# Dorothy-2016/rgbd360

Measured on AMD Instinct MI355X. Metric: registered Frame360 pairs/sec @ 8×640×480; ICP-reduce HBM GB/s vs roofline, higher is better.
Workload: dtype f32

## Files before the change

### include/rgbd360_hip.h

```cpp
#ifndef RGBD360_HIP_H
#define RGBD360_HIP_H
#include <stddef.h>
#include <stdint.h>

#ifdef __cplusplus
extern "C" {
#endif

#define R360_NUM_SENSORS 8
#define R360_MAX_PYR 6

typedef struct r360_ctx r360_ctx;
typedef struct r360_calib r360_calib;
typedef struct r360_frame r360_frame;

int         r360_ctx_create(int device, r360_ctx** out);
void        r360_ctx_destroy(r360_ctx* ctx);
int         r360_ctx_sync(r360_ctx* ctx);
void*       r360_ctx_stream(r360_ctx* ctx);
const char* r360_last_error(void);
const char* r360_version(void);
const char* r360_data_dir(void);

int  r360_calib_create(r360_ctx* ctx, int rows, int cols, r360_calib** out);
void r360_calib_destroy(r360_calib* c);
int  r360_calib_set_extrinsics(r360_calib* c, const float* rt8);
int  r360_calib_get_extrinsics(const r360_calib* c, float* rt8, float* rt_inv8, float K[9]);
int  r360_calib_load_extrinsics(r360_calib* c, const char* dir);
int  r360_calib_load_intrinsics(r360_calib* c, const char* dir);
int  r360_calib_create_sphere(r360_ctx* ctx, int sph_rows, int sph_cols, r360_calib** out);

enum {
    R360_BUILD_UNDISTORT = 1u << 0,
    R360_BUILD_SPHERE    = 1u << 1,
    R360_BUILD_PYRAMID   = 1u << 2,
    R360_BUILD_CLOUD     = 1u << 3,
    R360_BUILD_PLANES    = 1u << 4,
    R360_BUILD_SENSOR_PYRAMID = 1u << 5,
};
int  r360_frame_create(r360_ctx* ctx, const r360_calib* calib, r360_frame** out);
void r360_frame_destroy(r360_frame* f);
int  r360_frame_upload(r360_frame* f, const uint8_t* bgr8, const uint16_t* depth8);
int  r360_frame_upload_async(r360_frame* f, const uint8_t* bgr8, const uint16_t* depth8);
int  r360_frame_set_sphere(r360_frame* f, const uint8_t* bgr, const uint16_t* range_mm, int sph_rows, int sph_cols);
int  r360_host_register(void* p, size_t bytes);
int  r360_host_unregister(void* p);
int  r360_frame_upload_device(r360_frame* f, const void* d_bgr8, const void* d_depth8);
int  r360_frame_load_bin(r360_frame* f, const char* path);
int  r360_frame_save_bin(r360_frame* f, const char* path);
int  r360_frame_set_timestamp(r360_frame* f, uint64_t ts);
int  r360_frame_get_timestamp(const r360_frame* f, uint64_t* ts);
int  r360_frame_build(r360_frame* f, unsigned flags);
int  r360_frame_build_async(r360_frame* f, unsigned flags);
int  r360_frames_build(r360_frame* const* frames, int n, unsigned flags);
int  r360_frame_dims(const r360_frame* f, int* rows, int* cols, int* sph_rows, int* sph_cols);
int  r360_frame_set_levels(r360_frame* f, int n);
int  r360_frame_set_compaction(r360_frame* f, int all);
int  r360_frame_built(const r360_frame* f, unsigned* flags);
int  r360_frame_get_sphere(r360_frame* f, uint8_t* bgr, uint16_t* depth);
int  r360_frame_get_depth_m(r360_frame* f, float* depth8);
int  r360_frame_get_level(r360_frame* f, int level, int* rows, int* cols, float* gray, float* depth,
                          float* gx, float* gy, float* dgx, float* dgy);
int  r360_frame_get_points(r360_frame* f, int level, float* xyzg, int cap, int* n);
int  r360_frame_get_sensor_level(r360_frame* f, int sensor, int level, int* rows, int* cols, float* gray,
                                 float* depth, float* gx, float* gy, float* dgx, float* dgy);

enum { R360_PHOTO_CONSISTENCY = 0, R360_DEPTH_CONSISTENCY = 1, R360_PHOTO_DEPTH = 2 };

typedef struct {
    int    n_pyr;
    int    max_iters;
    float  min_depth;
    float  max_depth;
    float  std_dev_photo;
    float  std_dev_depth;
    float  thres_sal_int;
    float  thres_sal_depth;
    double tol_residual;
    double tol_update;
    double lambda;
    int    fixed_iters_level0;
} r360_icp_params;

typedef struct {
    int    iters[8];
    int    evals[8];
    int    illposed;
    float  sso;
    double error;
    int    passes;
    int    persistent;
    double av_photo_residual;
    double av_depth_residual;
    float  av_residual;
    int    residuals_set;
} r360_icp_stats;

void r360_icp_default_params(r360_icp_params* p);

int r360_align360(r360_ctx* ctx, r360_frame* trg, r360_frame* src, const float init[16],
                  int method, int occlusion, const r360_icp_params* p,
                  float pose_out[16], float H_out[36], float g_out[6], r360_icp_stats* st);
int r360_align360_async(r360_ctx* ctx, r360_frame* trg, r360_frame* src, const float init[16],
                        int method, int occlusion, const r360_icp_params* p);
int r360_align360_result(r360_ctx* ctx, float pose_out[16], float H_out[36], float g_out[6],
                         r360_icp_stats* st);

#define R360_MAX_BATCH_ALIGN 16
int r360_align360_batch_async(r360_ctx* ctx, int n, r360_frame* const* trg, r360_frame* const* src,
                              const float* init, int method, const r360_icp_params* p);
int r360_align360_batch_result(r360_ctx* ctx, float* pose_out, float* H_out, float* g_out, r360_icp_stats* st);

typedef struct r360_dense_queue r360_dense_queue;
int  r360_dense_queue_create(int device, int max_batch, r360_dense_queue** out);
void r360_dense_queue_destroy(r360_dense_queue* q);
r360_ctx* r360_dense_queue_ctx(r360_dense_queue* q);
int  r360_dense_queue_stats(r360_dense_queue* q, long* batches, long* jobs, int* max_batch_seen);
int  r360_dense_queue_submit(r360_dense_queue* q, r360_frame* trg, r360_frame* src, const float init[16],
                             int method, const r360_icp_params* p, long* ticket);
int  r360_dense_queue_collect(r360_dense_queue* q, long ticket, float pose_out[16], float H_out[36],
                              float g_out[6], r360_icp_stats* st);

int r360_icp_eval(r360_ctx* ctx, r360_frame* trg, r360_frame* src, int level, const float pose[16],
                  int method, const r360_icp_params* p, double H[36], double g[6],
                  double* err2, int* n_valid, int* n_visible);
int r360_icp_eval_occ(r360_ctx* ctx, r360_frame* trg, r360_frame* src, int level, const float pose[16],
                      int method, int occlusion, const r360_icp_params* p, double H[36], double g[6],
                      double* error, int* n_valid, int* n_visible);

int r360_align_pinhole(r360_ctx* ctx, r360_frame* trg, r360_frame* src, int sensor, const float init[16],
                       int method, const float* K, const r360_icp_params* p, float pose_out[16], float H_out[36],
                       float g_out[6], r360_icp_stats* st);
int r360_align_pinhole_async(r360_ctx* ctx, r360_frame* trg, r360_frame* src, int n, const int* sensors,
                             const float* init, int method, const float* K, const r360_icp_params* p);
int r360_align_pinhole_result(r360_ctx* ctx, float* poses, float* H, float* g, r360_icp_stats* st);
int r360_pinhole_eval(r360_ctx* ctx, r360_frame* trg, r360_frame* src, int sensor, int level, const float pose[16],
                      int method, const float* K, const r360_icp_params* p, double H[36], double g[6],
                      double* error, double res[2], int counts[3]);

typedef struct {
    double error[8];
    int    ran[8];
    int    n_visible[8];
    int    n_error[8];
    int    illposed_level;
    int    levels;
    int    info_set;
    int    pad;
    float  gradient[6];
} r360_dense_stats;
int r360_register_dense(r360_ctx* ctx, r360_frame* frame1, r360_frame* frame2, const float pose_estim[16],
                        int method, int mode, const r360_icp_params* p, float pose_out[16], float info_out[36],
                        r360_dense_stats* st);
int r360_dense_robot_eval(r360_ctx* ctx, r360_frame* frame1, r360_frame* frame2, int level, const float pose[16],
                          int method, const r360_icp_params* p, double err[16], double H[8 * 36], double g[8 * 6],
                          int counts[8 * 3]);

void r360_exp_se3(const double mu[6], int pseudo, float T[16]);

typedef struct {
    float normal[3], center[3], d, area, elongation, curvature, ppal[3], nrgb[3], intensity;
    int   id, sensor, n_inliers, n_hull;
} r360_plane;

int r360_frame_get_planes(r360_frame* f, r360_plane* out, int cap, int* n);
int r360_frame_set_plane_label(r360_frame* f, int i, const char* label);
int r360_frame_get_plane_label(r360_frame* f, int i, char* buf, int cap);
int r360_frame_get_plane_hull(r360_frame* f, int i, float* xyz, int cap, int* n);

int r360_frame_get_sphere_cloud(r360_frame* f, float* xyz, uint32_t* rgba, size_t cap, int* width, int* height);
int r360_pcd_write(const char* path, const float* xyz, const uint32_t* rgba, int width, int height, int mode);
int r360_pcd_read(const char* path, float* xyz, uint32_t* rgba, size_t cap, size_t* n, int* width, int* height);
int r360_frame_save_cloud(r360_frame* f, const char* path, int mode);
int r360_frame_load_cloud(r360_frame* f, const char* path);
int r360_frame_save_planes(r360_frame* f, const char* path);
int r360_frame_load_pbmap(r360_frame* f, const char* path);
int r360_frame_save(r360_frame* f, const char* dir, unsigned index);
int r360_frame_load_pbmap_cloud(r360_frame* f, const char* dir, unsigned index);

enum { R360_DEFAULT_6DoF = 0, R360_PLANAR_3DoF = 1, R360_ODOMETRY_6DoF = 2, R360_PLANAR_ODOMETRY_3DoF = 3 };

typedef struct {
    int   min_planes_recognition;
    float dist_d;
    float angle;
    float color_threshold;
    float intensity_threshold;
    float elongation_threshold;
    float area_threshold;
    float dist_threshold;
    float angle_threshold;
// ... 163 lines not shown
```

### rgbd360_amd/__init__.py

```python
from __future__ import annotations

import ctypes as C
import os
import numpy as np

C = C

__all__ = [
    "lib", "Context", "Calib360", "Frame360", "RegisterPhotoICP", "RegisterRGBD360", "IcpParams", "IcpStats",
    "PHOTO_CONSISTENCY", "DEPTH_CONSISTENCY", "PHOTO_DEPTH", "synth_path_pose", "exp_se3",
    "LIB_PATH", "ABI_SYMBOLS", "Batch", "PairJob", "PairResult", "JOB_PBMAP_ONLY", "JOB_GATED", "JOB_ALWAYS",
]

_HERE = os.path.dirname(os.path.abspath(__file__))
LIB_PATH = os.environ.get("R360_LIB") or os.path.join(_HERE, "lib", "librgbd360_hip.so")
REPO_ROOT = os.path.dirname(_HERE)

PHOTO_CONSISTENCY, DEPTH_CONSISTENCY, PHOTO_DEPTH = 0, 1, 2
BUILD_UNDISTORT, BUILD_SPHERE, BUILD_PYRAMID, BUILD_CLOUD, BUILD_PLANES = 1, 2, 4, 8, 16
BUILD_SENSOR_PYRAMID = 32
PCD_ASCII, PCD_BINARY, PCD_BINARY_COMPRESSED = 0, 1, 2


class IcpParams(C.Structure):
    _fields_ = [
        ("n_pyr", C.c_int), ("max_iters", C.c_int), ("min_depth", C.c_float), ("max_depth", C.c_float),
        ("std_dev_photo", C.c_float), ("std_dev_depth", C.c_float), ("thres_sal_int", C.c_float),
        ("thres_sal_depth", C.c_float), ("tol_residual", C.c_double), ("tol_update", C.c_double),
        ("lambda_", C.c_double), ("fixed_iters_level0", C.c_int),
    ]

    @classmethod
    def default(cls) -> "IcpParams":
        p = cls()
        lib().r360_icp_default_params(C.byref(p))
        return p


class MatchParams(C.Structure):
    _fields_ = [("min_planes_recognition", C.c_int), ("dist_d", C.c_float), ("angle", C.c_float),
                ("color_threshold", C.c_float), ("intensity_threshold", C.c_float),
                ("elongation_threshold", C.c_float), ("area_threshold", C.c_float), ("dist_threshold", C.c_float),
                ("angle_threshold", C.c_float), ("height_threshold", C.c_float), ("cos_angle_parallel", C.c_float),
                ("planar_normal_angle", C.c_float), ("max_nodes", C.c_long)]

    @classmethod
    def default(cls) -> "MatchParams":
        m = cls()
        lib().r360_match_params_default(C.byref(m))
        return m

    @classmethod
    def load_ini(cls, path: str, base: "MatchParams | None" = None) -> "MatchParams":
        m = cls.default() if base is None else base
        _check(lib().r360_match_params_load_ini(path.encode(), C.byref(m)), "match_params_load_ini")
        return m


class IcpStats(C.Structure):
    _fields_ = [
        ("iters", C.c_int * 8), ("evals", C.c_int * 8), ("illposed", C.c_int), ("sso", C.c_float),
        ("error", C.c_double), ("passes", C.c_int), ("persistent", C.c_int),
        ("av_photo_residual", C.c_double), ("av_depth_residual", C.c_double), ("av_residual", C.c_float),
        ("residuals_set", C.c_int),
    ]


class PairJob(C.Structure):
    _fields_ = [("ref", C.c_void_p), ("trg", C.c_void_p), ("dense", C.c_int), ("ref_is_source", C.c_int),
                ("guess", C.c_float * 16)]


class PairResult(C.Structure):
    _fields_ = [("good", C.c_int), ("n_match", C.c_int), ("area_matched", C.c_float), ("area_src", C.c_float),
                ("area_trg", C.c_float), ("sso_pbmap", C.c_float), ("pbmap_pose", C.c_float * 16),
                ("pbmap_info", C.c_float * 36), ("dense_rc", C.c_int), ("pose", C.c_float * 16),
                ("hessian", C.c_float * 36), ("stats", IcpStats)]

    def as_dict(self) -> dict:
        return {"good": self.good, "n_match": self.n_match, "area_matched": self.area_matched,
                "area_src": self.area_src, "area_trg": self.area_trg, "sso_pbmap": self.sso_pbmap,
                "pbmap_pose": _from16(np.array(self.pbmap_pose, np.float32)),
                "pbmap_info": np.array(self.pbmap_info, np.float32).reshape(6, 6).T.copy(),
                "dense_rc": self.dense_rc, "pose": _from16(np.array(self.pose, np.float32)),
                "hessian": np.array(self.hessian, np.float32).reshape(6, 6).T.copy(),
                "sso": self.stats.sso, "error": self.stats.error}


JOB_PBMAP_ONLY, JOB_GATED, JOB_ALWAYS = 0, 1, 2


class DenseStats(C.Structure):
    _fields_ = [("error", C.c_double * 8), ("ran", C.c_int * 8), ("n_visible", C.c_int * 8), ("n_error", C.c_int * 8),
                ("illposed_level", C.c_int), ("levels", C.c_int), ("info_set", C.c_int), ("pad", C.c_int),
                ("gradient", C.c_float * 6)]


class Plane(C.Structure):
    _fields_ = [("normal", C.c_float * 3), ("center", C.c_float * 3), ("d", C.c_float), ("area", C.c_float),
                ("elongation", C.c_float), ("curvature", C.c_float), ("ppal", C.c_float * 3), ("nrgb", C.c_float * 3),
                ("intensity", C.c_float), ("id", C.c_int), ("sensor", C.c_int), ("n_inliers", C.c_int),
                ("n_hull", C.c_int)]


class Region(C.Structure):
    _fields_ = [("label", C.c_int), ("count", C.c_int), ("start_idx", C.c_int), ("n_contour", C.c_int),
                ("n_fit", C.c_int), ("centroid", C.c_float * 3), ("cov", C.c_float * 9), ("model", C.c_float * 4),
                ("curvature", C.c_float)]


DEFAULT_6DoF, PLANAR_3DoF, ODOMETRY_6DoF, PLANAR_ODOMETRY_3DoF = 0, 1, 2, 3


_P = C.c_void_p
_FP = C.POINTER(C.c_float)
_DP = C.POINTER(C.c_double)
_IP = C.POINTER(C.c_int)
_SIGS = [
    ("r360_ctx_create", C.c_int, [C.c_int, C.POINTER(_P)]),
    ("r360_ctx_destroy", None, [_P]),
    ("r360_ctx_sync", C.c_int, [_P]),
    ("r360_ctx_stream", _P, [_P]),
    ("r360_last_error", C.c_char_p, []),
    ("r360_version", C.c_char_p, []),
    ("r360_calib_create", C.c_int, [_P, C.c_int, C.c_int, C.POINTER(_P)]),
    ("r360_calib_destroy", None, [_P]),
    ("r360_calib_set_extrinsics", C.c_int, [_P, _FP]),
    ("r360_calib_get_extrinsics", C.c_int, [_P, _FP, _FP, _FP]),
    ("r360_calib_load_extrinsics", C.c_int, [_P, C.c_char_p]),
    ("r360_calib_load_intrinsics", C.c_int, [_P, C.c_char_p]),
    ("r360_frame_create", C.c_int, [_P, _P, C.POINTER(_P)]),
    ("r360_frame_destroy", None, [_P]),
    ("r360_frame_upload", C.c_int, [_P, _P, _P]),
    ("r360_frame_upload_device", C.c_int, [_P, _P, _P]),
    ("r360_frame_upload_async", C.c_int, [_P, _P, _P]),
    ("r360_frame_set_sphere", C.c_int, [_P, _P, _P, C.c_int, C.c_int]),
    ("r360_calib_create_sphere", C.c_int, [_P, C.c_int, C.c_int, C.POINTER(_P)]),
    ("r360_host_register", C.c_int, [_P, C.c_size_t]),
    ("r360_host_unregister", C.c_int, [_P]),
    ("r360_frame_load_bin", C.c_int, [_P, C.c_char_p]),
    ("r360_frame_save_bin", C.c_int, [_P, C.c_char_p]),
    ("r360_frame_set_timestamp", C.c_int, [_P, C.c_uint64]),
    ("r360_frame_get_timestamp", C.c_int, [_P, C.POINTER(C.c_uint64)]),
    ("r360_frame_get_sphere_cloud", C.c_int, [_P, _FP, _P, C.c_size_t, _IP, _IP]),
    ("r360_pcd_write", C.c_int, [C.c_char_p, _FP, _P, C.c_int, C.c_int, C.c_int]),
    ("r360_pcd_read", C.c_int, [C.c_char_p, _FP, _P, C.c_size_t, C.POINTER(C.c_size_t), _IP, _IP]),
    ("r360_frame_save_cloud", C.c_int, [_P, C.c_char_p, C.c_int]),
    ("r360_frame_load_cloud", C.c_int, [_P, C.c_char_p]),
    ("r360_frame_save_planes", C.c_int, [_P, C.c_char_p]),
    ("r360_frame_load_pbmap", C.c_int, [_P, C.c_char_p]),
    ("r360_frame_save", C.c_int, [_P, C.c_char_p, C.c_uint]),
    ("r360_frame_load_pbmap_cloud", C.c_int, [_P, C.c_char_p, C.c_uint]),
    ("r360_frame_set_plane_label", C.c_int, [_P, C.c_int, C.c_char_p]),
    ("r360_frame_get_plane_label", C.c_int, [_P, C.c_int, C.c_char_p, C.c_int]),
    ("r360_frame_build", C.c_int, [_P, C.c_uint]),
    ("r360_frame_build_async", C.c_int, [_P, C.c_uint]),
    ("r360_frames_build", C.c_int, [_P, C.c_int, C.c_uint]),
    ("r360_frame_dims", C.c_int, [_P, _IP, _IP, _IP, _IP]),
    ("r360_frame_set_levels", C.c_int, [_P, C.c_int]),
    ("r360_frame_set_compaction", C.c_int, [_P, C.c_int]),
    ("r360_frame_built", C.c_int, [_P, C.POINTER(C.c_uint)]),
    ("r360_frame_get_sphere", C.c_int, [_P, _P, _P]),
    ("r360_frame_get_depth_m", C.c_int, [_P, _P]),
    ("r360_frame_get_level", C.c_int, [_P, C.c_int, _IP, _IP, _P, _P, _P, _P, _P, _P]),
    ("r360_frame_get_points", C.c_int, [_P, C.c_int, _FP, C.c_int, _IP]),
    ("r360_frame_get_sensor_level", C.c_int, [_P, C.c_int, C.c_int, _IP, _IP, _P, _P, _P, _P, _P, _P]),
    ("r360_icp_default_params", None, [C.POINTER(IcpParams)]),
    ("r360_align360", C.c_int, [_P, _P, _P, _FP, C.c_int, C.c_int, C.POINTER(IcpParams), _FP, _FP, _FP,
                                C.POINTER(IcpStats)]),
    ("r360_align360_async", C.c_int, [_P, _P, _P, _FP, C.c_int, C.c_int, C.POINTER(IcpParams)]),
    ("r360_align360_result", C.c_int, [_P, _FP, _FP, _FP, C.POINTER(IcpStats)]),
    ("r360_align360_batch_async", C.c_int, [_P, C.c_int, C.POINTER(C.c_void_p), C.POINTER(C.c_void_p), _FP, C.c_int,
                                            C.POINTER(IcpParams)]),
# ... 286 lines not shown
        c.h, c.ctx, c.rows, c.cols = h, ctx, rows, cols
        c.close = lambda: None
        return c

    @classmethod
    def for_sphere(cls, ctx: Context, sph_rows: int, sph_cols: int) -> "Calib360":
        return cls(ctx, _sphere=(sph_rows, sph_cols))

    def loadExtrinsicCalibration(self, path: str):
        _check(lib().r360_calib_load_extrinsics(self.h, path.encode()), "loadExtrinsicCalibration")

    def loadIntrinsicCalibration(self, path: str):
        _check(lib().r360_calib_load_intrinsics(self.h, path.encode()), "loadIntrinsicCalibration")

    def setRt(self, rt8: np.ndarray):
        a = np.concatenate([_mat16(m) for m in rt8]).astype(np.float32)
        _check(lib().r360_calib_set_extrinsics(self.h, _fptr(a)), "setRt")

    def extrinsics(self):
        rt = np.zeros(128, np.float32)
        rti = np.zeros(128, np.float32)
        K = np.zeros(9, np.float32)
        _check(lib().r360_calib_get_extrinsics(self.h, _fptr(rt), _fptr(rti), _fptr(K)), "get_extrinsics")
        return rt, rti, K

    def synth_frame(self, seed: int, rig_pose: np.ndarray):
        bgr = np.zeros((8, self.rows, self.cols, 3), np.uint8)
        dep = np.zeros((8, self.rows, self.cols), np.uint16)
        p = _mat16(rig_pose)
        _check(lib().r360_synth_frame(self.h, seed, _fptr(p), _vptr(bgr), _vptr(dep)), "synth_frame")
        return bgr, dep

    def close(self):
        if self.h:
            lib().r360_calib_destroy(self.h)
            self.h = None

    def __del__(self):
        try:
            self.close()
        except Exception:
            pass


class Frame360:

    def __init__(self, calib: Calib360):
        h = C.c_void_p()
        _check(lib().r360_frame_create(calib.ctx.h, calib.h, C.byref(h)), "r360_frame_create")
        self.h, self.calib = h, calib
        r, c, sr, sc = C.c_int(), C.c_int(), C.c_int(), C.c_int()
        lib().r360_frame_dims(h, C.byref(r), C.byref(c), C.byref(sr), C.byref(sc))
        self.rows, self.cols, self.sph_rows, self.sph_cols = r.value, c.value, sr.value, sc.value

    @classmethod
    def _view(cls, h, calib: Calib360) -> "Frame360":
        f = cls.__new__(cls)
        f.h, f.calib = h, calib
        r, c, sr, sc = C.c_int(), C.c_int(), C.c_int(), C.c_int()
        lib().r360_frame_dims(h, C.byref(r), C.byref(c), C.byref(sr), C.byref(sc))
        f.rows, f.cols, f.sph_rows, f.sph_cols = r.value, c.value, sr.value, sc.value
        f.close = lambda: None
        return f

    def setNumPyr(self, n: int):
        _check(lib().r360_frame_set_levels(self.h, int(n)), "r360_frame_set_levels")

    def setCompaction(self, all_levels: bool):
        _check(lib().r360_frame_set_compaction(self.h, int(bool(all_levels))), "r360_frame_set_compaction")

    def loadFrame(self, path: str):
        _check(lib().r360_frame_load_bin(self.h, path.encode()), "loadFrame")

    def serialize(self, fileName: str):
        _check(lib().r360_frame_save_bin(self.h, fileName.encode()), "serialize")

    def setTimeStamp(self, timestamp: int):
        _check(lib().r360_frame_set_timestamp(self.h, int(timestamp)), "setTimeStamp")

    @property
    def timeStamp(self) -> int:
        t = C.c_uint64()
        _check(lib().r360_frame_get_timestamp(self.h, C.byref(t)), "timeStamp")
        return t.value

    def sphereCloud(self):
        w, h = C.c_int(), C.c_int()
        _check(lib().r360_frame_get_sphere_cloud(self.h, None, None, 0, C.byref(w), C.byref(h)), "sphereCloud")
        n = w.value * h.value
        xyz = np.zeros((n, 3), np.float32)
        rgba = np.zeros(n, np.uint32)
        _check(lib().r360_frame_get_sphere_cloud(self.h, _fptr(xyz), _vptr(rgba), n, C.byref(w), C.byref(h)),
               "sphereCloud")
        return xyz, rgba, w.value, h.value

    def loadCloud(self, pointCloudPath: str):
        _check(lib().r360_frame_load_cloud(self.h, pointCloudPath.encode()), "loadCloud")

    def loadPbMap(self, pbmapPath: str):
        _check(lib().r360_frame_load_pbmap(self.h, pbmapPath.encode()), "loadPbMap")

    def load_PbMap_Cloud(self, path: str, index_or_pbmap):
        if isinstance(index_or_pbmap, str):
            self.loadCloud(path)
            self.loadPbMap(index_or_pbmap)
        else:
            _check(lib().r360_frame_load_pbmap_cloud(self.h, path.encode(), int(index_or_pbmap)), "load_PbMap_Cloud")

    def savePlanes(self, pathPbMap: str):
        _check(lib().r360_frame_save_planes(self.h, pathPbMap.encode()), "savePlanes")

    def saveCloud(self, path: str, mode: int = PCD_ASCII):
        _check(lib().r360_frame_save_cloud(self.h, path.encode(), mode), "saveCloud")

    def save(self, path: str, frame: int):
        _check(lib().r360_frame_save(self.h, path.encode(), int(frame)), "save")

    def setPlaneLabel(self, i: int, label: str):
        _check(lib().r360_frame_set_plane_label(self.h, i, label.encode()), "setPlaneLabel")

    def planeLabel(self, i: int) -> str:
        n = lib().r360_frame_get_plane_label(self.h, i, None, 0)
        _check(min(n, 0), "planeLabel")
        buf = C.create_string_buffer(n + 1)
        lib().r360_frame_get_plane_label(self.h, i, buf, n + 1)
        return buf.value.decode()

    def upload(self, bgr8: np.ndarray, depth8: np.ndarray):
        bgr8 = np.ascontiguousarray(bgr8, np.uint8)
        depth8 = np.ascontiguousarray(depth8, np.uint16)
        assert bgr8.shape == (8, self.rows, self.cols, 3) and depth8.shape == (8, self.rows, self.cols)
        _check(lib().r360_frame_upload(self.h, _vptr(bgr8), _vptr(depth8)), "upload")

    def set_sphere(self, bgr: np.ndarray, range_mm: np.ndarray):
        bgr = np.ascontiguousarray(bgr, np.uint8)
        range_mm = np.ascontiguousarray(range_mm, np.uint16)
        H, W = range_mm.shape
        assert bgr.shape == (H, W, 3)
        _check(lib().r360_frame_set_sphere(self.h, _vptr(bgr), _vptr(range_mm), H, W), "set_sphere")

    def upload_async(self, bgr8: np.ndarray, depth8: np.ndarray):
        assert bgr8.dtype == np.uint8 and depth8.dtype == np.uint16
        assert bgr8.flags.c_contiguous and depth8.flags.c_contiguous
        assert bgr8.shape == (8, self.rows, self.cols, 3) and depth8.shape == (8, self.rows, self.cols)
        _check(lib().r360_frame_upload_async(self.h, _vptr(bgr8), _vptr(depth8)), "upload_async")

    def upload_device(self, d_bgr: int, d_depth: int):
        _check(lib().r360_frame_upload_device(self.h, C.c_void_p(d_bgr), C.c_void_p(d_depth)), "upload_device")

    def build(self, flags: int = BUILD_UNDISTORT | BUILD_SPHERE | BUILD_PYRAMID, sync: bool = True):
        fn = lib().r360_frame_build if sync else lib().r360_frame_build_async
        _check(fn(self.h, flags), "r360_frame_build")

    def undistort(self):
        self.build(BUILD_UNDISTORT)

    def stitchSphericalImage(self):
        self.build(BUILD_SPHERE | BUILD_PYRAMID)

    def buildSphereCloud(self):
        self.build(BUILD_UNDISTORT | BUILD_CLOUD)

    def getPlanes(self):
        self.build(BUILD_UNDISTORT | BUILD_PLANES)
        return self.planes()

    def planes(self) -> list[dict]:
        n = C.c_int()
        _check(lib().r360_frame_get_planes(self.h, None, 0, C.byref(n)), "get_planes")
        arr = (Plane * max(n.value, 1))()
        _check(lib().r360_frame_get_planes(self.h, arr, n.value, C.byref(n)), "get_planes")
        out = []
        for i, p in enumerate(arr[:n.value]):
            hull = np.zeros((max(p.n_hull, 1), 3), np.float32)
            m = C.c_int()
            _check(lib().r360_frame_get_plane_hull(self.h, i, _fptr(hull), p.n_hull, C.byref(m)), "get_plane_hull")
            out.append(dict(normal=np.array(p.normal[:]), center=np.array(p.center[:]), d=p.d, area=p.area,
                            elongation=p.elongation, curvature=p.curvature, ppal=np.array(p.ppal[:]),
                            nrgb=np.array(p.nrgb[:]), intensity=p.intensity, id=p.id, sensor=p.sensor,
                            n_inliers=p.n_inliers, hull=hull[:p.n_hull].copy()))
        return out

    def cloud(self):
        h, w = self.rows // 2, self.cols // 2
        xyz = np.zeros((8, h, w, 4), np.float32)
        rgb = np.zeros((8, h, w, 4), np.uint8)
        nrm = np.zeros((8, h, w, 4), np.float32)
        dist = np.zeros((8, h, w), np.float32)
        _check(lib().r360_frame_get_cloud(self.h, _fptr(xyz), _vptr(rgb), _fptr(nrm), _fptr(dist)), "get_cloud")
        return xyz, rgb, nrm, dist

    def labels(self):
        h, w = self.rows // 2, self.cols // 2
        lab = np.zeros((8, h, w), np.int32)
        labf = np.zeros((8, h, w), np.int32)
        _check(lib().r360_frame_get_labels(self.h, lab.ctypes.data_as(_IP), labf.ctypes.data_as(_IP)), "get_labels")
        return lab, labf

    def regions(self, sensor: int) -> list[dict]:
        n = C.c_int()
        arr = (Region * 64)()
        _check(lib().r360_frame_get_regions(self.h, sensor, arr, 64, C.byref(n)), "get_regions")
        return [dict(label=r.label, count=r.count, start_idx=r.start_idx, n_contour=r.n_contour, n_fit=r.n_fit,
                     centroid=np.array(r.centroid[:]), cov=np.array(r.cov[:]).reshape(3, 3),
                     model=np.array(r.model[:]), curvature=r.curvature) for r in arr[:n.value]]

    def sphere(self):
        bgr = np.zeros((self.sph_rows, self.sph_cols, 3), np.uint8)
        dep = np.zeros((self.sph_rows, self.sph_cols), np.uint16)
        _check(lib().r360_frame_get_sphere(self.h, _vptr(bgr), _vptr(dep)), "get_sphere")
        return bgr, dep

    def depth_m(self):
        d = np.zeros((8, self.rows, self.cols), np.float32)
        _check(lib().r360_frame_get_depth_m(self.h, _vptr(d)), "get_depth_m")
        return d

    def level(self, level: int):
        r, c = C.c_int(), C.c_int()
        _check(lib().r360_frame_get_level(self.h, level, C.byref(r), C.byref(c), None, None, None, None, None,
                                          None), "get_level")
        arrs = [np.zeros((r.value, c.value), np.float32) for _ in range(6)]
        _check(lib().r360_frame_get_level(self.h, level, C.byref(r), C.byref(c), *[_vptr(a) for a in arrs]),
               "get_level")
        return dict(zip(["gray", "depth", "gx", "gy", "dgx", "dgy"], arrs))

    def points(self, level: int) -> np.ndarray:
        n = C.c_int()
        _check(lib().r360_frame_get_points(self.h, level, None, 0, C.byref(n)), "get_points")
        out = np.zeros((max(n.value, 1), 4), np.float32)
        _check(lib().r360_frame_get_points(self.h, level, _fptr(out), n.value, C.byref(n)), "get_points")
        return out[:n.value]

    def sensor_level(self, sensor: int, level: int):
        r, c = C.c_int(), C.c_int()
        _check(lib().r360_frame_get_sensor_level(self.h, sensor, level, C.byref(r), C.byref(c), None, None, None,
                                                 None, None, None), "get_sensor_level")
        arrs = [np.zeros((r.value, c.value), np.float32) for _ in range(6)]
        _check(lib().r360_frame_get_sensor_level(self.h, sensor, level, C.byref(r), C.byref(c),
                                                 *[_vptr(a) for a in arrs]), "get_sensor_level")
        return dict(zip(["gray", "depth", "gx", "gy", "dgx", "dgy"], arrs))

    def close(self):
        if self.h:
            lib().r360_frame_destroy(self.h)
            self.h = None

    def __del__(self):
        try:
            self.close()
        except Exception:
            pass


class RegisterRGBD360:

    def __init__(self, ctx: "Context", config_file: str | None = None):
        self.ctx = ctx
        self.config_file = config_file
        self.match = MatchParams.load_ini(config_file) if config_file else MatchParams.default()
        self.rigidTransf = np.eye(4, dtype=np.float32)
        self.informationM = np.zeros((6, 6), np.float32)
        self.bestMatch: dict[int, int] = {}
        self.areaMatched = self.areaSource = self.areaTarget = 0.0
        self.ref = self.trg = None
        self.max_match_planes = 0

    def setReference(self, ref: "Frame360", max_match_planes: int = 0):
        self.ref, self.max_match_planes = ref, max_match_planes

    def setTarget(self, trg: "Frame360", max_match_planes: int = 0):
        self.trg, self.max_match_planes = trg, max_match_planes

    def RegisterPbMap(self, frame1=None, frame2=None, max_match_planes: int = 0, registMode: int = DEFAULT_6DoF) -> bool:
        if frame1 is not None:
            self.setReference(frame1, max_match_planes)
        if frame2 is not None:
            self.setTarget(frame2, max_match_planes)
        pose = _mat16(self.rigidTransf)
        info = np.ascontiguousarray(self.informationM.T).reshape(36).copy()
        pairs = np.zeros(512, np.int32)
        n = C.c_int()
        am, as_, at = C.c_float(), C.c_float(self.areaSource), C.c_float(self.areaTarget)
        _check(lib().r360_ctx_set_match_params(self.ctx.h, C.byref(self.match)), "set_match_params")
        rc = _check(lib().r360_register_pbmap(self.ctx.h, self.ref.h, self.trg.h, self.max_match_planes, registMode,
                                              _fptr(pose), _fptr(info), pairs.ctypes.data_as(_IP), 256, C.byref(n),
                                              C.byref(am), C.byref(as_), C.byref(at)), "RegisterPbMap")
        self.bestMatch = {int(pairs[2 * k]): int(pairs[2 * k + 1]) for k in range(min(n.value, 256))}
        self.areaMatched = am.value
        if rc == 1:
            self.rigidTransf = _from16(pose)
            self.informationM = info.reshape(6, 6).T.copy()
            self.areaSource, self.areaTarget = as_.value, at.value
        return rc == 1

    def RegisterDensePhotoICP(self, frame1, frame2, pose_estim=None, method: int = PHOTO_CONSISTENCY,
                              registMode: int = DEFAULT_6DoF, params: "IcpParams | None" = None) -> bool:
        init = _mat16(np.eye(4) if pose_estim is None else pose_estim)
        po = np.zeros(16, np.float32)
        info = np.ascontiguousarray(self.informationM.T).reshape(36).copy()
        self.dense_stats = DenseStats()
        rc = _check(lib().r360_register_dense(self.ctx.h, frame1.h, frame2.h, _fptr(init), method, registMode,
                                              None if params is None else C.byref(params), _fptr(po), _fptr(info),
                                              C.byref(self.dense_stats)), "RegisterDensePhotoICP")
        self.rigidTransf = _from16(po)
        if rc == 1:
# ... 502 lines not shown
```

### rgbd360_amd/csrc/host/runtime.cpp

```cpp
#include <atomic>
#include <chrono>
#include <dlfcn.h>
#include <mutex>
#include <unordered_map>
#include <sys/prctl.h>
#include <cmath>
#include <thread>
#include <cstdarg>
#include <cstdio>
#include <cstring>
#include <fstream>
#include <sstream>
#include <string>
#include <vector>

#include "../r360_internal.h"

static thread_local std::string g_err;
void r360_set_error(const char* fmt, ...) {
    char buf[1024];
    va_list ap;
    va_start(ap, fmt);
    vsnprintf(buf, sizeof(buf), fmt, ap);
    va_end(ap);
// ... 520 lines not shown
extern "C" int r360_frame_create(r360_ctx* ctx, const r360_calib* calib, r360_frame** out) {
    CHECK_ARG(ctx && calib && out, "null arg");
    R360_HIP(hipSetDevice(ctx->device));
    r360_frame* f = new r360_frame;
    f->ctx = ctx; f->calib = calib;
    f->rows = calib->rows; f->cols = calib->cols;
    f->sph_rows = calib->sph_rows; f->sph_cols = calib->sph_cols;
    f->n_levels = calib->n_levels;
    const size_t ns = (size_t)8 * f->rows * f->cols, nsph = (size_t)f->sph_rows * f->sph_cols;
    if (ns) {
        R360_HIP(hipMalloc(&f->d_bgr, ns * 3));
        R360_HIP(hipMalloc(&f->d_depth, ns * 2));
        R360_HIP(hipMalloc(&f->d_depth_m, ns * 4));
    }
    R360_HIP(hipMalloc(&f->d_sph_bgr, nsph * 3));
    R360_HIP(hipMalloc(&f->d_sph_depth, nsph * 2));
    int R = f->sph_rows, C = f->sph_cols;
    for (int l = 0; l < f->n_levels; ++l) {
        f->lv[l].rows = R; f->lv[l].cols = C;
        R360_HIP(hipMalloc(&f->lv[l].p0, sizeof(float2) * (size_t)R * C));
        R360_HIP(hipMalloc(&f->lv[l].tg, sizeof(float4) * (size_t)R * C));
        R360_HIP(hipMalloc(&f->lv[l].pts, sizeof(float4) * (size_t)R * C));
        if (l == 0) R360_HIP(hipMalloc(&f->lv[l].pk, sizeof(uint32_t) * (size_t)R * C));
        R /= 2; C /= 2;
    }
    f->src_blocks = (int)((nsph + R360_SRC_BLOCK - 1) / R360_SRC_BLOCK);
    R360_HIP(hipMalloc(&f->d_npts, sizeof(int) * R360_MAX_PYR));
    R360_HIP(hipMemsetAsync(f->d_npts, 0, sizeof(int) * R360_MAX_PYR, f->ctx->stream));
    R360_HIP(hipMalloc(&f->d_src_cnt, sizeof(int) * R360_MAX_PYR * (size_t)f->src_blocks));
    SrcLevel sl[R360_MAX_PYR];
    for (int l = 0; l < f->n_levels; ++l) {
        const LevelTrig& T = calib->trig[l];
        sl[l] = SrcLevel{f->lv[l].p0, f->lv[l].pts, T.sinphi, T.cosphi, T.sinth, T.costh, f->lv[l].rows, f->lv[l].cols};
    }
    R360_HIP(hipMalloc(&f->d_src_levels, sizeof(SrcLevel) * R360_MAX_PYR));
    R360_HIP(hipMemcpy(f->d_src_levels, sl, sizeof(SrcLevel) * f->n_levels, hipMemcpyHostToDevice));
    R360_HIP(hipEventCreateWithFlags(&f->bgr_ev, hipEventDisableTiming));
    *out = f;
    return 0;
}

static std::mutex g_bev_m;
static std::unordered_map<const r360_frame*, hipEvent_t> g_bev;

hipEvent_t frame_build_event(const r360_frame* f) {
    std::lock_guard<std::mutex> lk(g_bev_m);
    auto it = g_bev.find(f);
    return it == g_bev.end() ? nullptr : it->second;
}

static int frame_build_event_record(const r360_frame* f) {
    hipEvent_t e = nullptr;
    {
        std::lock_guard<std::mutex> lk(g_bev_m);
        auto it = g_bev.find(f);
        if (it != g_bev.end()) e = it->second;
    }
    if (!e) {
        R360_HIP(hipEventCreateWithFlags(&e, hipEventDisableTiming));
        std::lock_guard<std::mutex> lk(g_bev_m);
        g_bev[f] = e;
    }
    R360_HIP(hipEventRecord(e, f->ctx->stream));
    const_cast<r360_frame*>(f)->build_gen.fetch_add(1, std::memory_order_release);
    return 0;
}

extern "C" void r360_frame_destroy(r360_frame* f) {
    if (!f) return;
    {
        std::lock_guard<std::mutex> lk(g_bev_m);
        auto it = g_bev.find(f);
        if (it != g_bev.end()) {
            (void)hipEventDestroy(it->second);
            g_bev.erase(it);
        }
    }
    hipFree(f->d_bgr); hipFree(f->d_depth); hipFree(f->d_depth_m); hipFree(f->d_sph_bgr); hipFree(f->d_sph_depth);
    for (int l = 0; l < R360_MAX_PYR; ++l) { hipFree(f->lv[l].p0); hipFree(f->lv[l].tg); hipFree(f->lv[l].pts); hipFree(f->lv[l].pk); }
    hipFree(f->d_npts); hipFree(f->d_src_cnt); hipFree(f->d_src_levels);
    for (int l = 0; l < f->n_slevels; ++l) { hipFree(f->sp[l].p0); hipFree(f->sp[l].tg); }
    plane_bufs_free(f);
    if (f->bgr_ev) hipEventDestroy(f->bgr_ev);
    delete f->sphere_cloud;
    delete f;
}

static int frame_copy_images(r360_frame* f, const void* bgr8, const void* depth8, hipMemcpyKind kind) {
    r360_ctx* ctx = f->ctx;
    const size_t ns = (size_t)8 * f->rows * f->cols;
    if (ctx->split_upload) {
        R360_HIP(hipMemcpyAsync(f->d_depth, depth8, ns * 2, kind, ctx->stream));
        if (!ctx->up_stream) {
            R360_HIP(hipStreamCreateWithFlags(&ctx->up_stream, hipStreamNonBlocking));
            R360_HIP(hipEventCreateWithFlags(&ctx->up_ev, hipEventDisableTiming));
        }
        R360_HIP(hipEventRecord(ctx->up_ev, ctx->stream));
        R360_HIP(hipStreamWaitEvent(ctx->up_stream, ctx->up_ev, 0));
        R360_HIP(hipMemcpyAsync(f->d_bgr, bgr8, ns * 3, kind, ctx->up_stream));
        R360_HIP(hipEventRecord(f->bgr_ev, ctx->up_stream));
        f->bgr_split = true;
    } else {
        if (hipEvent_t e = f->bgr_wait()) R360_HIP(hipStreamWaitEvent(ctx->stream, e, 0));
        R360_HIP(hipMemcpyAsync(f->d_bgr, bgr8, ns * 3, kind, ctx->stream));
        R360_HIP(hipMemcpyAsync(f->d_depth, depth8, ns * 2, kind, ctx->stream));
        f->bgr_split = false;
    }
    return 0;
}

extern "C" int r360_frame_upload(r360_frame* f, const uint8_t* bgr8, const uint16_t* depth8) {
    CHECK_ARG(f && bgr8 && depth8, "null arg");
    if (f && bind_device(f->ctx->device)) return -1;
    CHECK_ARG(f->rows > 0, "a sphere-only frame has no sensor images");
    planes_join(f);
    if (frame_copy_images(f, bgr8, depth8, hipMemcpyHostToDevice)) return -1;
    R360_HIP(hipStreamSynchronize(f->ctx->stream));
    if (hipEvent_t e = f->bgr_wait()) R360_HIP(hipEventSynchronize(e));
    f->built = 0;
    return 0;
}

extern "C" int r360_frame_upload_async(r360_frame* f, const uint8_t* bgr8, const uint16_t* depth8) {
    CHECK_ARG(f && bgr8 && depth8, "null arg");
    if (f && bind_device(f->ctx->device)) return -1;
    CHECK_ARG(f->rows > 0, "a sphere-only frame has no sensor images");
    planes_join(f);
    if (frame_copy_images(f, bgr8, depth8, hipMemcpyHostToDevice)) return -1;
    f->built = 0;
    return 0;
}

extern "C" int r360_host_register(void* p, size_t bytes) {
    CHECK_ARG(p && bytes, "null arg");
    R360_HIP(hipHostRegister(p, bytes, hipHostRegisterDefault));
    return 0;
}

extern "C" int r360_host_unregister(void* p) {
    CHECK_ARG(p, "null arg");
    R360_HIP(hipHostUnregister(p));
    return 0;
}

extern "C" int r360_frame_set_sphere(r360_frame* f, const uint8_t* bgr, const uint16_t* range_mm, int sph_rows,
                                     int sph_cols) {
    CHECK_ARG(f && bgr && range_mm, "null arg");
    if (f && bind_device(f->ctx->device)) return -1;
    CHECK_ARG(sph_rows == f->sph_rows && sph_cols == f->sph_cols,
              "sphere size differs from the frame's (create it from r360_calib_create_sphere)");
    const size_t n = (size_t)sph_rows * sph_cols;
    R360_HIP(hipMemcpyAsync(f->d_sph_bgr, bgr, n * 3, hipMemcpyHostToDevice, f->ctx->stream));
    R360_HIP(hipMemcpyAsync(f->d_sph_depth, range_mm, n * 2, hipMemcpyHostToDevice, f->ctx->stream));
    if (launch_sphere_level0(f) || launch_pyramid(f) || frame_build_event_record(f)) return -1;
    R360_HIP(hipStreamSynchronize(f->ctx->stream));
    f->built = (f->built & ~(unsigned)(R360_BUILD_SPHERE | R360_BUILD_PYRAMID)) | R360_BUILD_SPHERE | R360_BUILD_PYRAMID;
    return 0;
}

extern "C" int r360_frame_upload_device(r360_frame* f, const void* d_bgr8, const void* d_depth8) {
    CHECK_ARG(f && d_bgr8 && d_depth8, "null arg");
    if (f && bind_device(f->ctx->device)) return -1;
    CHECK_ARG(f->rows > 0, "a sphere-only frame has no sensor images");
    planes_join(f);
    const size_t ns = (size_t)8 * f->rows * f->cols;
    if (hipEvent_t e = f->bgr_wait()) R360_HIP(hipStreamWaitEvent(f->ctx->stream, e, 0));
    R360_HIP(hipMemcpyAsync(f->d_bgr, d_bgr8, ns * 3, hipMemcpyDeviceToDevice, f->ctx->stream));
    f->bgr_split = false;
    R360_HIP(hipMemcpyAsync(f->d_depth, d_depth8, ns * 2, hipMemcpyDeviceToDevice, f->ctx->stream));
    f->built = 0;
    return 0;
}

extern "C" int r360_frame_build_async(r360_frame* f, unsigned flags) {
    CHECK_ARG(f, "null frame");
    if (f && bind_device(f->ctx->device)) return -1;
    CHECK_ARG(f->rows > 0 || flags == 0, "a sphere-only frame has no sensor images to build from (r360_frame_set_sphere)");
    if (flags & (R360_BUILD_UNDISTORT | R360_BUILD_CLOUD | R360_BUILD_PLANES)) {
        planes_join(f);
        if (launch_undistort(f)) return -1;
        f->built |= R360_BUILD_UNDISTORT;
    }
    if (flags & (R360_BUILD_CLOUD | R360_BUILD_PLANES)) {
        if (planes_enqueue(f)) return -1;
        f->built |= R360_BUILD_CLOUD | R360_BUILD_PLANES;
        delete f->sphere_cloud;
        f->sphere_cloud = nullptr;
    }
    if (flags & (R360_BUILD_SPHERE | R360_BUILD_PYRAMID)) {
        if (launch_stitch(f)) return -1;
        f->built |= R360_BUILD_SPHERE;
    }
    if (flags & R360_BUILD_PYRAMID) {
        if (launch_pyramid(f)) return -1;
        f->built |= R360_BUILD_PYRAMID;
        if (frame_build_event_record(f)) return -1;
    }
    if (flags & R360_BUILD_SENSOR_PYRAMID) {
        if (launch_sensor_pyramid(f)) return -1;
        f->built |= R360_BUILD_SENSOR_PYRAMID;
    }
    return 0;
}

extern "C" int r360_frame_build(r360_frame* f, unsigned flags) {
    int rc = r360_frame_build_async(f, flags);
    if (rc) return rc;
    if (flags & R360_BUILD_PLANES) return planes_finish(f);
    R360_HIP(hipStreamSynchronize(f->ctx->stream));
    return 0;
}

extern "C" int r360_frame_set_levels(r360_frame* f, int n) {
    CHECK_ARG(f && f->calib, "null frame");
    CHECK_ARG(n >= 1 && n <= f->calib->n_levels, "levels must be 1 .. the calibration's pyramid depth");
    planes_join(f);
    f->n_levels = n;
    f->built = 0;
    return 0;
}

extern "C" int r360_frame_set_compaction(r360_frame* f, int all) {
    CHECK_ARG(f, "null frame");
    f->compact_all = all != 0;
    return 0;
}

extern "C" int r360_frame_dims(const r360_frame* f, int* rows, int* cols, int* sph_rows, int* sph_cols) {
    CHECK_ARG(f, "null frame");
    if (rows) *rows = f->rows;
    if (cols) *cols = f->cols;
    if (sph_rows) *sph_rows = f->sph_rows;
    if (sph_cols) *sph_cols = f->sph_cols;
    return 0;
}

extern "C" int r360_frame_built(const r360_frame* f, unsigned* flags) {
    CHECK_ARG(f && flags, "null arg");
    *flags = f->built.load();
    return 0;
}

extern "C" int r360_frame_get_sphere(r360_frame* f, uint8_t* bgr, uint16_t* depth) {
    CHECK_ARG(f, "null frame");
    CHECK_ARG(f->built & R360_BUILD_SPHERE, "sphere not built");
    const size_t n = (size_t)f->sph_rows * f->sph_cols;
    R360_HIP(hipStreamSynchronize(f->ctx->stream));
    if (bgr) R360_HIP(hipMemcpy(bgr, f->d_sph_bgr, n * 3, hipMemcpyDeviceToHost));
    if (depth) R360_HIP(hipMemcpy(depth, f->d_sph_depth, n * 2, hipMemcpyDeviceToHost));
    return 0;
}

extern "C" int r360_frame_get_depth_m(r360_frame* f, float* depth8) {
    CHECK_ARG(f && depth8, "null arg");
    CHECK_ARG(f->built & R360_BUILD_UNDISTORT, "undistorted depth not built");
    R360_HIP(hipStreamSynchronize(f->ctx->stream));
    R360_HIP(hipMemcpy(depth8, f->d_depth_m, sizeof(float) * 8 * f->rows * f->cols, hipMemcpyDeviceToHost));
    return 0;
}

static int copy_level(r360_frame* f, const float2* d_p0, const float4* d_tg, int R, int C, int* rows, int* cols,
                      float* gray, float* depth, float* gx, float* gy, float* dgx, float* dgy) {
    if (rows) *rows = R;
    if (cols) *cols = C;
    const size_t n = (size_t)R * C;
    R360_HIP(hipStreamSynchronize(f->ctx->stream));
    std::vector<float2> p0(n);
    std::vector<float4> tg(n);
    R360_HIP(hipMemcpy(p0.data(), d_p0, n * sizeof(float2), hipMemcpyDeviceToHost));
    R360_HIP(hipMemcpy(tg.data(), d_tg, n * sizeof(float4), hipMemcpyDeviceToHost));
    for (size_t i = 0; i < n; ++i) {
        if (gray) gray[i] = p0[i].x;
        if (depth) depth[i] = p0[i].y;
        if (gx) gx[i] = tg[i].x;
        if (gy) gy[i] = tg[i].y;
        if (dgx) dgx[i] = tg[i].z;
        if (dgy) dgy[i] = tg[i].w;
    }
    return 0;
}

extern "C" int r360_frame_get_level(r360_frame* f, int level, int* rows, int* cols, float* gray, float* depth,
                                    float* gx, float* gy, float* dgx, float* dgy) {
    CHECK_ARG(f, "null frame");
    CHECK_ARG(level >= 0 && level < f->n_levels, "level out of range");
    CHECK_ARG(f->built & R360_BUILD_PYRAMID, "pyramid not built");
    const LevelBufs& L = f->lv[level];
    return copy_level(f, L.p0, L.tg, L.rows, L.cols, rows, cols, gray, depth, gx, gy, dgx, dgy);
}

extern "C" int r360_frame_get_points(r360_frame* f, int level, float* xyzg, int cap, int* n) {
    CHECK_ARG(f && n, "null arg");
    CHECK_ARG(level >= 0 && level < f->n_levels, "level out of range");
    CHECK_ARG(f->built & R360_BUILD_PYRAMID, "pyramid not built");
    if (!((f->compacted >> level) & 1u)) {
        if (int rc = launch_src_compaction(f, 1u << level)) return rc;
        f->compacted |= 1u << level;
    }
    int np = 0;
    R360_HIP(hipMemcpyAsync(&np, f->d_npts + level, sizeof(int), hipMemcpyDeviceToHost, f->ctx->stream));
    R360_HIP(hipStreamSynchronize(f->ctx->stream));
    *n = np;
    if (xyzg && cap > 0) {
        const int m = np < cap ? np : cap;
        R360_HIP(hipMemcpy(xyzg, f->lv[level].pts, sizeof(float4) * (size_t)m, hipMemcpyDeviceToHost));
    }
    return 0;
}

extern "C" int r360_frame_get_sensor_level(r360_frame* f, int sensor, int level, int* rows, int* cols, float* gray,
                                           float* depth, float* gx, float* gy, float* dgx, float* dgy) {
    CHECK_ARG(f, "null frame");
    CHECK_ARG(f->built & R360_BUILD_SENSOR_PYRAMID, "sensor pyramid not built (R360_BUILD_SENSOR_PYRAMID)");
    CHECK_ARG(level >= 0 && level < f->n_slevels, "level out of range");
    CHECK_ARG(sensor >= 0 && sensor < 8, "sensor out of range");
    const LevelBufs& L = f->sp[level];
    const size_t off = (size_t)sensor * L.rows * L.cols;
    return copy_level(f, L.p0 + off, L.tg + off, L.rows, L.cols, rows, cols, gray, depth, gx, gy, dgx, dgy);
}

extern "C" void r360_icp_default_params(r360_icp_params* p) {
    p->n_pyr = 4;
    p->max_iters = 10;
    p->min_depth = 0.3f;
    p->max_depth = 6.0f;
    p->std_dev_photo = (float)(6. / 255);
    p->std_dev_depth = 0.2f;
    p->thres_sal_int = 0.01f;
    p->thres_sal_depth = 0.01f;
    p->tol_residual = 1e-3;
    p->tol_update = 1e-4;
    p->lambda = 1.0;
    p->fixed_iters_level0 = 0;
}

static IcpConst make_const(const r360_icp_params* p, int level, int n_pixels, int occ = 0) {
    IcpConst C;
    memset(&C, 0, sizeof(C));
    C.min_d = p->min_depth; C.max_d = p->max_depth;
    C.sd_photo = p->std_dev_photo; C.sd_depth = p->std_dev_depth;
    C.thr_int = p->thres_sal_int; C.thr_depth = p->thres_sal_depth;
    C.sd_photo_inv_f = (float)(1. / p->std_dev_photo);
    C.sd_photo_inv_d = 1. / p->std_dev_photo;
    C.tol_res = p->tol_residual; C.tol_upd = p->tol_update; C.lambda = p->lambda;
    C.max_iters = p->max_iters; C.fixed_iters0 = p->fixed_iters_level0;
    static const int diag_extra = R360_KNOB("R360_DIAG_EXTRA_ITERS", 0);
    if (C.fixed_iters0 > 0) C.fixed_iters0 += diag_extra;
    C.n_pixels = n_pixels; C.level = level; C.occ = occ;
    return C;
}

static int check_pair(r360_ctx* ctx, r360_frame* trg, r360_frame* src, const r360_icp_params* p) {
    CHECK_ARG(ctx && trg && src && p, "null arg");
    CHECK_ARG(trg->sph_rows == src->sph_rows && trg->sph_cols == src->sph_cols, "frame size mismatch");
    CHECK_ARG((trg->built & R360_BUILD_PYRAMID) && (src->built & R360_BUILD_PYRAMID),
              "frames need R360_BUILD_PYRAMID (setSourceFrame/setTargetFrame)");
    CHECK_ARG(p->n_pyr >= 1 && p->n_pyr <= src->n_levels, "n_pyr exceeds the frame's pyramid depth");
    CHECK_ARG(p->min_depth == 0.3f && p->max_depth == 6.0f,
              "non-default min/max depth changes the depth pyramid: not supported in this version");
    CHECK_ARG(ctx->partials_cap >= icp_blocks_for(src->lv[0].rows * src->lv[0].cols), "partials buffer too small");
    return 0;
}

template <class Enqueue>
static int align_graph_launch(r360_ctx* ctx, const r360_frame* trg, const r360_frame* src, int method,
                              const r360_icp_params* p, bool persist, Enqueue&& enqueue) {
    std::vector<uintptr_t> key;
    key.reserve(16 + 20 * p->n_pyr);
    auto put = [&](const void* q) { key.push_back((uintptr_t)q); };
    put(trg); put(src); key.push_back((uintptr_t)method); key.push_back((uintptr_t)persist);
    put(ctx->d_state); put(ctx->d_partials); put(ctx->d_gticket); put(ctx->d_defer);
    key.push_back((uintptr_t)ctx->defer_cap); key.push_back((uintptr_t)ctx->partials_cap); put(ctx->d_ktime);
    put(src->d_npts); put(src->calib);
    {
        uintptr_t w[(sizeof(r360_icp_params) + sizeof(uintptr_t) - 1) / sizeof(uintptr_t)] = {};
        memcpy(w, p, sizeof(r360_icp_params));
        for (uintptr_t x : w) key.push_back(x);
    }
    for (int l = 0; l < p->n_pyr; ++l) {
        for (const r360_frame* f : {trg, src}) {
            const LevelBufs& L = f->lv[l];
            key.push_back(((uintptr_t)(unsigned)L.rows << 32) | (unsigned)L.cols);
            put(L.p0); put(L.tg); put(L.pts); put(L.pk);
        }
        const LevelTrig& T = src->calib->trig[l];
        put(T.sinphi); put(T.cosphi); put(T.sinth); put(T.costh);
    }
    ++ctx->graph_clock;
    for (auto& g : ctx->graphs)
        if (g.key == key) {
            g.used = ctx->graph_clock;
            R360_HIP(hipGraphLaunch(g.exec, ctx->stream));
            return 0;
        }
    hipGraph_t graph = nullptr;
    hipStream_t cs = capture_stream(ctx);
    if (!cs) return -1;
    hipStream_t own = ctx->stream;
    R360_HIP(hipStreamBeginCapture(cs, hipStreamCaptureModeRelaxed));
    ctx->stream = cs;
    const int rc = enqueue();
    ctx->stream = own;
    const hipError_t ec = hipStreamEndCapture(cs, &graph);
    if (rc) { if (graph) (void)hipGraphDestroy(graph); return rc; }
    R360_HIP(ec);
    hipGraphExec_t exec = nullptr;
    const hipError_t ei = hipGraphInstantiate(&exec, graph, nullptr, nullptr, 0);
    (void)hipGraphDestroy(graph);
    R360_HIP(ei);
    constexpr size_t kMaxGraphs = 8;
    if (ctx->graphs.size() >= kMaxGraphs) {
        size_t lru = 0;
        for (size_t i = 1; i < ctx->graphs.size(); ++i)
            if (ctx->graphs[i].used < ctx->graphs[lru].used) lru = i;
        R360_HIP(hipStreamSynchronize(ctx->stream));
        (void)hipGraphExecDestroy(ctx->graphs[lru].exec);
        ctx->graphs.erase(ctx->graphs.begin() + (long)lru);
    }
    ctx->graphs.push_back({std::move(key), exec, ctx->graph_clock});
    R360_HIP(hipGraphLaunch(exec, ctx->stream));
    return 0;
}

static std::atomic<int> g_persist_slot{0};
static bool persist_take(r360_ctx* ctx) {
    if (ctx->persist_held) return true;
    int z = 0;
    if (!g_persist_slot.compare_exchange_strong(z, 1)) return false;
    ctx->persist_held = 1;
    return true;
}
void persist_release(r360_ctx* ctx) {
    if (!ctx->persist_held) return;
    ctx->persist_held = 0;
    g_persist_slot.store(0);
}

extern "C" int r360_align360_async(r360_ctx* ctx, r360_frame* trg, r360_frame* src, const float init[16], int method,
                                   int occlusion, const r360_icp_params* p) {
    if (ctx && bind_device(ctx->device)) return -1;
    if (int rc = check_pair(ctx, trg, src, p)) return rc;
    CHECK_ARG(init, "null init pose");
    CHECK_ARG(method >= 0 && method <= 2, "invalid method");
    CHECK_ARG(occlusion >= 0 && occlusion <= 2, "occlusion must be 0, 1 or 2");
    if (ensure_defer(ctx, src->lv[0].rows * src->lv[0].cols)) return -1;
    for (const r360_frame* f : {trg, src})
        if (f->ctx != ctx)
            if (hipEvent_t e = frame_build_event(f)) R360_HIP(hipStreamWaitEvent(ctx->stream, e, 0));
    IcpState* h = ctx->h_state;
    ctx->align_t0 = now_s();
    memset(h, 0, sizeof(IcpState));
    memcpy(h->pose, init, sizeof(float) * 16);
    memcpy(h->cand, init, sizeof(float) * 16);
    h->dbg[8] = ~0ull;
    R360_HIP(hipMemcpyAsync(ctx->d_state, h, sizeof(IcpState), hipMemcpyHostToDevice, ctx->stream));
    static const bool persist_env = R360_KNOB("R360_PERSIST", 0) != 0;
    static const int persist_min = R360_KNOB("R360_PERSIST_MIN_LEVEL", 0);
    bool persist = (ctx->persist_levels || persist_env) && !occlusion && !ctx->timing && !R360_POLL;
    for (int l = persist_min; persist && l < p->n_pyr; ++l) persist = icp_level_persist_ok(ctx, src, l, method);
    if (persist) persist = persist_take(ctx);
    auto passes_of = [&]() -> int {
        for (int l = p->n_pyr - 1; l >= 0; --l) {
            const int np = src->lv[l].rows * src->lv[l].cols;
            const IcpConst C = make_const(p, l, np, occlusion);
            const int passes = 1 + ((l == 0 && p->fixed_iters_level0 > 0) ? p->fixed_iters_level0 : p->max_iters);
            if (persist && l >= persist_min) {
                if (launch_icp_level_persist(ctx, trg, src, l, method, C, passes)) return -1;
                continue;
            }
            for (int k = 0; k < passes; ++k)
                if (launch_icp_level(ctx, trg, src, l, method, C, k == 0, 0)) return -1;
        }
        return 0;
    };
    static const bool no_graph = R360_KNOB("R360_NO_GRAPH", 0) != 0;
    int rc;
    if (no_graph || R360_POLL || occlusion || ctx->timing) rc = passes_of();
    else rc = align_graph_launch(ctx, trg, src, method, p, persist, passes_of);
    if (rc) {
        persist_release(ctx);
        return -1;
    }
    ctx->async_nL = p->n_pyr;
    ctx->async_persist = persist ? 1 : 0;
    ctx->async_pending = 1;
    return 0;
}

static void fill_stats(const IcpState* h, r360_icp_stats* st) {
    memset(st, 0, sizeof(*st));
    for (int l = 0; l < 8; ++l) { st->iters[l] = h->iters[l]; st->evals[l] = h->evals_l[l]; }
    st->illposed = h->illposed;
    st->sso = h->sso;
    st->error = h->error;
    st->passes = h->passes;
    st->av_photo_residual = h->av_photo;
    st->av_depth_residual = h->av_depth;
    st->av_residual = h->av_res;
    st->residuals_set = h->av_set & 3;
}

extern "C" int r360_align360_result(r360_ctx* ctx, float pose_out[16], float H_out[36], float g_out[6],
                                    r360_icp_stats* st) {
    CHECK_ARG(ctx && ctx->async_pending, "no alignment pending");
    IcpState* h = ctx->h_state;
    R360_HIP(hipMemcpyAsync(h, ctx->d_state, sizeof(IcpState), hipMemcpyDeviceToHost, ctx->stream));
    bool waited = false;
    const int wrc = align_wait(ctx, &waited);
    if (wrc == 0 && waited) ctx->align_est = now_s() - ctx->align_t0;
    persist_release(ctx);
    if (wrc) return -1;
    ctx->async_pending = 0;
    if (h->fault) {
        R360_HIP(hipMemsetAsync(ctx->d_gticket, 0, sizeof(unsigned) * R360_TICKET_STRIDE * R360_TICKET_GROUPS,
                                ctx->stream));
        R360_HIP(hipStreamSynchronize(ctx->stream));
        r360_set_error("alignFrames360: a persistent level launch timed out waiting for a pass (GPU oversubscribed?)");
        return -1;
    }
    if (pose_out) memcpy(pose_out, h->pose, sizeof(float) * 16);
    if (H_out) memcpy(H_out, h->Hout, sizeof(float) * 36);
    if (g_out) memcpy(g_out, h->gout, sizeof(float) * 6);
    if (st) {
        fill_stats(h, st);
        st->persistent = ctx->async_persist;
    }
    return h->illposed ? 1 : 0;
}

extern "C" int r360_align360(r360_ctx* ctx, r360_frame* trg, r360_frame* src, const float init[16], int method,
                             int occlusion, const r360_icp_params* p, float pose_out[16], float H_out[36],
                             float g_out[6], r360_icp_stats* st) {
    if (int rc = r360_align360_async(ctx, trg, src, init, method, occlusion, p)) return rc;
    return r360_align360_result(ctx, pose_out, H_out, g_out, st);
}

int align360_batch_enqueue(r360_ctx* ctx, int n, r360_frame* const* trg, r360_frame* const* src, const float* init,
                           int method, const r360_icp_params* p, bool wait_frames);

int ctx_wait_frames(r360_ctx* ctx, r360_frame* const* frames, int n) {
    std::vector<hipStream_t> seen;
    for (int i = 0; i < n; ++i) {
        hipStream_t s = frames[i]->ctx->stream;
        if (s == ctx->stream) continue;
        bool dup = false;
        for (hipStream_t t : seen) dup = dup || t == s;
        if (dup) continue;
        seen.push_back(s);
    }
    while (ctx->sync_ev.size() < seen.size()) {
        hipEvent_t e;
        R360_HIP(hipEventCreateWithFlags(&e, hipEventDisableTiming));
        ctx->sync_ev.push_back(e);
    }
    for (size_t i = 0; i < seen.size(); ++i) {
        R360_HIP(hipEventRecord(ctx->sync_ev[i], seen[i]));
        R360_HIP(hipStreamWaitEvent(ctx->stream, ctx->sync_ev[i], 0));
    }
    return 0;
}

extern "C" int r360_align360_batch_async(r360_ctx* ctx, int n, r360_frame* const* trg, r360_frame* const* src,
                                         const float* init, int method, const r360_icp_params* p) {
    if (ctx && bind_device(ctx->device)) return -1;
    return align360_batch_enqueue(ctx, n, trg, src, init, method, p, true);
}

int align360_batch_enqueue(r360_ctx* ctx, int n, r360_frame* const* trg, r360_frame* const* src, const float* init,
                           int method, const r360_icp_params* p, bool wait_frames) {
    CHECK_ARG(ctx && trg && src && init && p, "null arg");
    CHECK_ARG(n >= 1 && n <= R360_MAX_BATCH, "batch size must be 1..R360_MAX_BATCH");
    CHECK_ARG(!ctx->batch_pending, "a batch is pending on this ctx (r360_align360_batch_result)");
    CHECK_ARG(method >= 0 && method <= 2, "invalid method");
    for (int j = 0; j < n; ++j) {
        if (int rc = check_pair(ctx, trg[j], src[j], p)) return rc;
        CHECK_ARG(src[j]->sph_rows == src[0]->sph_rows && src[j]->sph_cols == src[0]->sph_cols,
                  "batched alignments need frames of one sphere size");
    }
    if (ensure_batch(ctx, n, (long)src[0]->lv[0].rows * src[0]->lv[0].cols)) return -1;
    std::vector<r360_frame*> fr;
    for (int j = 0; j < n; ++j) { fr.push_back(trg[j]); fr.push_back(src[j]); }
    if (wait_frames && ctx_wait_frames(ctx, fr.data(), 2 * n)) return -1;
    for (int j = 0; j < n; ++j) {
        IcpState* h = ctx->h_bstate + j;
        memset(h, 0, sizeof(IcpState));
        memcpy(h->pose, init + 16 * j, sizeof(float) * 16);
        memcpy(h->cand, init + 16 * j, sizeof(float) * 16);
        h->dbg[8] = ~0ull;
    }
    R360_HIP(hipMemcpyAsync(ctx->d_bstate, ctx->h_bstate, sizeof(IcpState) * n, hipMemcpyHostToDevice, ctx->stream));
    const size_t tk = (size_t)R360_TICKET_GROUPS * R360_TICKET_STRIDE;
    for (int l = p->n_pyr - 1; l >= 0; --l) {
        IcpJobs jobs;
        for (int j = 0; j < n; ++j) {
            IcpJob& J = jobs.j[j];
            J.src = src[j]->lv[l].p0; J.trg = trg[j]->lv[l].p0; J.tg = trg[j]->lv[l].tg;
            J.pts = src[j]->lv[l].pts; J.npts = src[j]->d_npts + l;
            J.spk = src[j]->lv[l].pk; J.tpk = trg[j]->lv[l].pk;
            J.S = ctx->d_bstate + j;
            J.partials = ctx->d_bpartials + (size_t)j * 32 * ctx->partials_cap;
            J.gcnt = ctx->d_bgticket + (size_t)j * tk;
            J.dq = ctx->d_bdefer + (size_t)j * ctx->bdefer_cap;
        }
        const int np = src[0]->lv[l].rows * src[0]->lv[l].cols;
        const IcpConst C = make_const(p, l, np, 0);
        const int passes = 1 + ((l == 0 && p->fixed_iters_level0 > 0) ? p->fixed_iters_level0 : p->max_iters);
        const int prc = launch_icp_levels_batch(ctx, jobs, n, src[0], l, method, C, passes);
        if (prc < 0) return prc;
        if (prc == 0) continue;
        for (int k = 0; k < passes; ++k)
            if (int rc = launch_icp_jobs(ctx, jobs, n, src[0], l, method, C, k == 0, 0)) return rc;
    }
    ctx->batch_n = n;
    ctx->batch_pending = 1;
    return 0;
}

extern "C" int r360_align360_batch_result(r360_ctx* ctx, float* pose_out, float* H_out, float* g_out,
                                          r360_icp_stats* st) {
    CHECK_ARG(ctx && ctx->batch_pending, "no batched alignment pending");
    const int n = ctx->batch_n;
    R360_HIP(hipMemcpyAsync(ctx->h_bstate, ctx->d_bstate, sizeof(IcpState) * n, hipMemcpyDeviceToHost, ctx->stream));
    if (ctx_wait(ctx)) return -1;
    ctx->batch_pending = 0;
    bool fault = false;
    for (int j = 0; j < n; ++j) fault = fault || ctx->h_bstate[j].fault;
    if (fault) {
        R360_HIP(hipMemsetAsync(ctx->d_bgticket, 0, sizeof(unsigned) * R360_TICKET_STRIDE * R360_TICKET_GROUPS * n,
                                ctx->stream));
        R360_HIP(hipStreamSynchronize(ctx->stream));
        r360_set_error("alignFrames360 batch: a persistent level launch timed out waiting for a pass (GPU oversubscribed?)");
        return -1;
    }
    int ill = 0;
    for (int j = 0; j < n; ++j) {
        const IcpState* h = ctx->h_bstate + j;
        if (pose_out) memcpy(pose_out + 16 * j, h->pose, sizeof(float) * 16);
        if (H_out) memcpy(H_out + 36 * j, h->Hout, sizeof(float) * 36);
        if (g_out) memcpy(g_out + 6 * j, h->gout, sizeof(float) * 6);
        if (st) fill_stats(h, st + j);
        ill += h->illposed ? 1 : 0;
    }
    return ill;
}

static int icp_eval_sums(r360_ctx* ctx, r360_frame* trg, r360_frame* src, int level, const float pose[16], int method,
                         int occ, const r360_icp_params* p, double sums[R360_NSUMS]) {
    if (int rc = check_pair(ctx, trg, src, p)) return rc;
    CHECK_ARG(level >= 0 && level < src->n_levels, "level out of range");
    CHECK_ARG(method >= 0 && method <= 2, "invalid method");
    CHECK_ARG(occ >= 0 && occ <= 2, "occlusion must be 0, 1 or 2");
    if (ensure_defer(ctx, src->lv[level].rows * src->lv[level].cols)) return -1;
    IcpState* h = ctx->h_state;
    memset(h, 0, sizeof(IcpState));
    memcpy(h->cand, pose, sizeof(float) * 16);
    memcpy(h->pose, pose, sizeof(float) * 16);
    h->dbg[8] = ~0ull;
    R360_HIP(hipMemcpyAsync(ctx->d_state, h, sizeof(IcpState), hipMemcpyHostToDevice, ctx->stream));
    const IcpConst C = make_const(p, level, src->lv[level].rows * src->lv[level].cols, occ);
    if (launch_icp_level(ctx, trg, src, level, method, C, 0, 1)) return -1;
    R360_HIP(hipMemcpyAsync(h, ctx->d_state, sizeof(IcpState), hipMemcpyDeviceToHost, ctx->stream));
    if (ctx_wait(ctx)) return -1;
    memcpy(sums, h->sums, sizeof(double) * R360_NSUMS);
    return 0;
}

static void sums_hg(const double* s, double H[36], double g[6]) {
    int k = 0;
    for (int u = 0; u < 6; ++u)
        for (int v = u; v < 6; ++v) { H[u * 6 + v] = H[v * 6 + u] = s[k++]; }
    for (int u = 0; u < 6; ++u) g[u] = s[21 + u];
}

extern "C" int r360_icp_eval(r360_ctx* ctx, r360_frame* trg, r360_frame* src, int level, const float pose[16],
                             int method, const r360_icp_params* p, double H[36], double g[6], double* err2,
                             int* n_valid, int* n_visible) {
    double s[R360_NSUMS];
    if (int rc = icp_eval_sums(ctx, trg, src, level, pose, method, 0, p, s)) return rc;
    sums_hg(s, H, g);
    if (err2) *err2 = s[R360_SUM_ERR2];
    if (n_valid) *n_valid = (int)s[R360_SUM_NVALID];
    if (n_visible) *n_visible = (int)s[R360_SUM_NVIS];
    return 0;
}

extern "C" int r360_icp_eval_occ(r360_ctx* ctx, r360_frame* trg, r360_frame* src, int level, const float pose[16],
                                 int method, int occlusion, const r360_icp_params* p, double H[36], double g[6],
                                 double* error, int* n_valid, int* n_visible) {
    double s[R360_NSUMS];
    if (int rc = icp_eval_sums(ctx, trg, src, level, pose, method, occlusion, p, s)) return rc;
    sums_hg(s, H, g);
    const double e2 = s[R360_SUM_ERR2], nv = s[R360_SUM_NVALID];
    if (error)
        *error = occlusion == 0 ? std::sqrt(e2 / nv)
               : occlusion == 1 ? std::sqrt(e2 / nv) + std::sqrt(s[R360_SUM_ERR2D] / s[R360_SUM_NDEPTH])
                                : std::sqrt(e2 / nv) + std::sqrt(s[R360_SUM_ERR2D] / nv);
    if (n_valid) *n_valid = (int)(nv + (occlusion == 1 ? s[R360_SUM_NDEPTH] : 0.0));
    if (n_visible) *n_visible = (int)s[R360_SUM_NVIS];
    return 0;
}

extern "C" void r360_exp_se3(const double mu[6], int pseudo, float T[16]) {
    const double wx = mu[3], wy = mu[4], wz = mu[5];
    const double th2 = wx * wx + wy * wy + wz * wz, th = std::sqrt(th2);
    double A, B, Cc;
    if (th < 1e-6) { A = 1 - th2 / 6; B = 0.5 - th2 / 24; Cc = 1.0 / 6 - th2 / 120; }
    else { A = std::sin(th) / th; B = (1 - std::cos(th)) / th2; Cc = (th - std::sin(th)) / (th2 * th); }
    const double W[9] = {0, -wz, wy, wz, 0, -wx, -wy, wx, 0};
    double W2[9];
    for (int r = 0; r < 3; ++r)
        for (int c = 0; c < 3; ++c) {
            double s = 0;
            for (int k = 0; k < 3; ++k) s += W[r * 3 + k] * W[k * 3 + c];
            W2[r * 3 + c] = s;
        }
    for (int c = 0; c < 4; ++c)
        for (int r = 0; r < 4; ++r) {
            double v;
            const double I = (r == c) ? 1.0 : 0.0;
            if (r < 3 && c < 3) v = I + A * W[r * 3 + c] + B * W2[r * 3 + c];
            else if (r < 3) {
                if (pseudo) v = mu[r];
                else {
                    v = 0;
                    for (int k = 0; k < 3; ++k) v += ((r == k ? 1.0 : 0.0) + B * W[r * 3 + k] + Cc * W2[r * 3 + k]) * mu[k];
                }
            } else v = (c == 3) ? 1.0 : 0.0;
            T[c * 4 + r] = (float)v;
        }
}

extern "C" int r360_ctx_debug_stamps(r360_ctx* ctx, unsigned long long* out12) {
    CHECK_ARG(ctx && out12, "null arg");
    R360_HIP(hipStreamSynchronize(ctx->stream));
    R360_HIP(hipMemcpy(out12, (const char*)ctx->d_state + offsetof(IcpState, dbg), sizeof(unsigned long long) * 12,
                       hipMemcpyDeviceToHost));
    return 0;
}
```

### rgbd360_amd/csrc/kernels/frame_kernels.hip

```cpp
#include "../r360_internal.h"

namespace {

constexpr int TPB = 256;

__global__ void k_undistort(const uint16_t* __restrict__ depth, float* __restrict__ depth_m, int rows, int cols,
                            const float* __restrict__ mult, const float* __restrict__ counts, int nx, int bin_w,
                            int bin_h, int nb, double bin_depth, int apply) {
    const long n = (long)R360_NUM_SENSORS * rows * cols;
    for (long i = blockIdx.x * (long)blockDim.x + threadIdx.x; i < n; i += (long)gridDim.x * blockDim.x) {
        float z = (float)depth[i] * 0.001f;
        if (apply && z != 0) {
            const int s = (int)(i / ((long)rows * cols));
            const int pix = (int)(i - (long)s * rows * cols);
            const int v = pix / cols, u = pix - v * cols;
            const long fr = ((long)s * (rows / bin_h) * nx + (long)(v / bin_h) * nx + (u / bin_w)) * nb;
            int idx = (int)floor(z / bin_depth);
            idx = idx < nb - 1 ? idx : nb - 1;
            float start = (float)(bin_depth * idx);
            int idx1 = (z - start < bin_depth / 2) ? idx : idx + 1;
            int idx0 = idx1 - 1;
            if (idx0 < 0 || idx1 >= nb || counts[fr + idx0] < 50 || counts[fr + idx1] < 50) {
                z *= mult[fr + idx];
            } else {
// ... 8 lines not shown
    }
}

__device__ __forceinline__ float undistort_px(float z, int s, int v, int u, int rows, int cols,
                                              const float* __restrict__ mult, const float* __restrict__ counts, int nx,
                                              int bin_w, int bin_h, int nb, double bin_depth) {
    const long fr = ((long)s * (rows / bin_h) * nx + (long)(v / bin_h) * nx + (u / bin_w)) * nb;
    int idx = (int)floor(z / bin_depth);
    idx = idx < nb - 1 ? idx : nb - 1;
    float start = (float)(bin_depth * idx);
    int idx1 = (z - start < bin_depth / 2) ? idx : idx + 1;
    int idx0 = idx1 - 1;
    if (idx0 < 0 || idx1 >= nb || counts[fr + idx0] < 50 || counts[fr + idx1] < 50) return z * mult[fr + idx];
    double z0 = (idx0 + 1) * bin_depth - bin_depth * 0.5;
    double c1 = (z - z0) / bin_depth;
    double c0 = 1.0 - c1;
    double m = c0 * mult[fr + idx0] + c1 * mult[fr + idx1];
    return (float)(z * m);
}

__global__ void k_undistort4(const uint16_t* __restrict__ depth, float* __restrict__ depth_m, int rows, int cols,
                             const float* __restrict__ mult, const float* __restrict__ counts, int nx, int bin_w,
                             int bin_h, int nb, double bin_depth, int apply) {
    const long nq = (long)R360_NUM_SENSORS * rows * cols / 4;
    for (long q = blockIdx.x * (long)blockDim.x + threadIdx.x; q < nq; q += (long)gridDim.x * blockDim.x) {
        const uint2 d4 = reinterpret_cast<const uint2*>(depth)[q];
        const unsigned dv[4] = {d4.x & 0xffffu, d4.x >> 16, d4.y & 0xffffu, d4.y >> 16};
        float z[4];
        const int pq = rows * cols / 4;
        const int qi = (int)q;
        const int s = qi / pq;
        const int pix = (qi - s * pq) * 4;
        const int v = pix / cols, u0 = pix - v * cols;
#pragma unroll
        for (int e = 0; e < 4; ++e) {
            z[e] = (float)dv[e] * 0.001f;
            if (apply && z[e] != 0)
                z[e] = undistort_px(z[e], s, v, u0 + e, rows, cols, mult, counts, nx, bin_w, bin_h, nb, bin_depth);
        }
        reinterpret_cast<float4*>(depth_m)[q] = make_float4(z[0], z[1], z[2], z[3]);
    }
}

__global__ void k_stitch(const uint8_t* __restrict__ bgr8, const uint16_t* __restrict__ depth8, int rows, int cols,
                         int H, int W, const float* __restrict__ sinphi, const float* __restrict__ cosphi,
                         const float* __restrict__ sinth, const float* __restrict__ costh,
                         const float* __restrict__ rt_inv, float fx, float fy, float cx, float cy,
                         uint8_t* __restrict__ sph_bgr, uint16_t* __restrict__ sph_depth, float2* __restrict__ p0,
                         uint32_t* __restrict__ pk) {
    const long n = (long)H * W;
    for (long i = blockIdx.x * (long)blockDim.x + threadIdx.x; i < n; i += (long)gridDim.x * blockDim.x) {
        const int row = (int)(i / W), col = (int)(i - (long)row * W);
        const int k = 7 - col / rows;
        const float* T = rt_inv + 16 * k;
        const float v0 = sinphi[row], cos_phi = cosphi[row];
        const float v1 = cos_phi * sinth[col];
        const float v2 = cos_phi * costh[col];
        float p0x = T[0] * v0 + T[4] * v1 + T[8] * v2;
        float p1 = T[1] * v0 + T[5] * v1 + T[9] * v2;
        float p2 = T[2] * v0 + T[6] * v1 + T[10] * v2;
        p0x = p0x + T[12]; p1 = p1 + T[13]; p2 = p2 + T[14];
        const float u = fx * p0x / p2 + cx;
        const float v = fy * p1 / p2 + cy;
        uint8_t b = 0, g = 0, r = 0;
        uint16_t dd = 0;
        if (u >= 0 && u < cols && v >= 0 && v < rows) {
            const int iu = (int)u, iv = (int)v;
            const long si = (long)k * rows * cols + (long)iv * cols + iu;
            b = bgr8[si * 3 + 0]; g = bgr8[si * 3 + 1]; r = bgr8[si * 3 + 2];
            const double du = (double)((u - cx) / fx), dv = (double)((v - cy) / fy);
            dd = (uint16_t)(depth8[si] * sqrt(1 + du * du + dv * dv));
        }
        sph_bgr[i * 3 + 0] = b; sph_bgr[i * 3 + 1] = g; sph_bgr[i * 3 + 2] = r;
        sph_depth[i] = dd;
        const int y = (b * 4899 + g * 9617 + r * 1868 + (1 << 13)) >> 14;
        p0[i] = make_float2((float)y * (float)(1. / 255), (float)dd * 0.001f);
        pk[i] = dd | ((unsigned)y << 16);
    }
}

__global__ void k_stitch4(const uint8_t* __restrict__ bgr8, const uint16_t* __restrict__ depth8, int rows, int cols,
                          int H, int W, const float* __restrict__ sinphi, const float* __restrict__ cosphi,
                          const float* __restrict__ sinth, const float* __restrict__ costh,
                          const float* __restrict__ rt_inv, float fx, float fy, float cx, float cy,
                          uint8_t* __restrict__ sph_bgr, uint16_t* __restrict__ sph_depth, float2* __restrict__ p0,
                          uint32_t* __restrict__ pk) {
    const long nq = (long)H * W / 4;
    for (long q = blockIdx.x * (long)blockDim.x + threadIdx.x; q < nq; q += (long)gridDim.x * blockDim.x) {
        const long i0 = 4 * q;
        const int row = (int)(i0 / W), col0 = (int)(i0 - (long)row * W);
        const float v0 = sinphi[row], cos_phi = cosphi[row];
        const float4 st4 = *reinterpret_cast<const float4*>(sinth + col0);
        const float4 ct4 = *reinterpret_cast<const float4*>(costh + col0);
        const float st_[4] = {st4.x, st4.y, st4.z, st4.w}, ct_[4] = {ct4.x, ct4.y, ct4.z, ct4.w};
        const int kA = 7 - col0 / rows;
        const bool one_sensor = kA == 7 - (col0 + 3) / rows;
        const float4* TA4 = reinterpret_cast<const float4*>(rt_inv + 16 * kA);
        const float4 ta0 = TA4[0], ta1 = TA4[1], ta2 = TA4[2], ta3 = TA4[3];
        const float TA[16] = {ta0.x, ta0.y, ta0.z, ta0.w, ta1.x, ta1.y, ta1.z, ta1.w,
                              ta2.x, ta2.y, ta2.z, ta2.w, ta3.x, ta3.y, ta3.z, ta3.w};
        unsigned char px[12];
        unsigned short dd4[4];
        unsigned pk4[4];
        float2 o[4];
#pragma unroll
        for (int e = 0; e < 4; ++e) {
            const int col = col0 + e;
            const int k = 7 - col / rows;
            float T[16];
            if (one_sensor) {
#pragma unroll
                for (int t = 0; t < 16; ++t) T[t] = TA[t];
            } else {
#pragma unroll
                for (int t = 0; t < 16; ++t) T[t] = rt_inv[16 * k + t];
            }
            const float v1 = cos_phi * st_[e];
            const float v2 = cos_phi * ct_[e];
            float p0x = T[0] * v0 + T[4] * v1 + T[8] * v2;
            float p1 = T[1] * v0 + T[5] * v1 + T[9] * v2;
            float p2 = T[2] * v0 + T[6] * v1 + T[10] * v2;
            p0x = p0x + T[12]; p1 = p1 + T[13]; p2 = p2 + T[14];
            const float u = fx * p0x / p2 + cx;
            const float v = fy * p1 / p2 + cy;
            uint8_t b = 0, g = 0, r = 0;
            uint16_t dd = 0;
            if (u >= 0 && u < cols && v >= 0 && v < rows) {
                const int iu = (int)u, iv = (int)v;
                const long si = (long)k * rows * cols + (long)iv * cols + iu;
                b = bgr8[si * 3 + 0]; g = bgr8[si * 3 + 1]; r = bgr8[si * 3 + 2];
                const double du = (double)((u - cx) / fx), dv = (double)((v - cy) / fy);
                dd = (uint16_t)(depth8[si] * sqrt(1 + du * du + dv * dv));
            }
            px[3 * e] = b; px[3 * e + 1] = g; px[3 * e + 2] = r;
            dd4[e] = dd;
            const int y = (b * 4899 + g * 9617 + r * 1868 + (1 << 13)) >> 14;
            o[e] = make_float2((float)y * (float)(1. / 255), (float)dd * 0.001f);
            pk4[e] = dd | ((unsigned)y << 16);
        }
        uint3 wb;
        wb.x = px[0] | (px[1] << 8) | (px[2] << 16) | ((unsigned)px[3] << 24);
        wb.y = px[4] | (px[5] << 8) | (px[6] << 16) | ((unsigned)px[7] << 24);
        wb.z = px[8] | (px[9] << 8) | (px[10] << 16) | ((unsigned)px[11] << 24);
        *reinterpret_cast<uint3*>(sph_bgr + 12 * q) = wb;
        *reinterpret_cast<uint2*>(sph_depth + i0) = make_uint2(dd4[0] | ((unsigned)dd4[1] << 16),
                                                                 dd4[2] | ((unsigned)dd4[3] << 16));
        *reinterpret_cast<float4*>(p0 + i0) = make_float4(o[0].x, o[0].y, o[1].x, o[1].y);
        *reinterpret_cast<float4*>(p0 + i0 + 2) = make_float4(o[2].x, o[2].y, o[3].x, o[3].y);
        *reinterpret_cast<uint4*>(pk + i0) = make_uint4(pk4[0], pk4[1], pk4[2], pk4[3]);
    }
}

constexpr int STT_R = 64, STT_C = 16;
__global__ void __launch_bounds__(256) k_stitch_t(const uint8_t* __restrict__ bgr8, const uint16_t* __restrict__ depth8,
                                                  int rows, int cols, int H, int W, const float* __restrict__ sinphi,
                                                  const float* __restrict__ cosphi, const float* __restrict__ sinth,
                                                  const float* __restrict__ costh, const float* __restrict__ rt_inv,
                                                  float fx, float fy, float cx, float cy, uint8_t* __restrict__ sph_bgr,
                                                  uint16_t* __restrict__ sph_depth, float2* __restrict__ p0,
                                                  uint32_t* __restrict__ pk) {
    __shared__ uint32_t s_pk[STT_C][STT_R + 1];
    __shared__ uint32_t s_bgr[STT_C][STT_R + 1];
    const int lane = threadIdx.x & 63, w = threadIdx.x >> 6;
    const int tiles_x = W / STT_C;
    const int tx = blockIdx.x % tiles_x, ty = blockIdx.x / tiles_x;
    const int row = ty * STT_R + lane;
    const bool in = row < H;
    const float v0 = in ? sinphi[row] : 0.f, cos_phi = in ? cosphi[row] : 0.f;
#pragma unroll
    for (int j = 0; j < STT_C / 4; ++j) {
        const int cl = w * (STT_C / 4) + j;
        const int col = __builtin_amdgcn_readfirstlane(tx * STT_C + cl);
        const int k = 7 - col / rows;
        const float* T = rt_inv + 16 * k;
        const float v1 = cos_phi * sinth[col];
        const float v2 = cos_phi * costh[col];
        float p0x = T[0] * v0 + T[4] * v1 + T[8] * v2;
        float p1 = T[1] * v0 + T[5] * v1 + T[9] * v2;
        float p2 = T[2] * v0 + T[6] * v1 + T[10] * v2;
        p0x = p0x + T[12]; p1 = p1 + T[13]; p2 = p2 + T[14];
        const float u = fx * p0x / p2 + cx;
        const float v = fy * p1 / p2 + cy;
        unsigned b = 0, g = 0, r = 0, dd = 0;
        if (in && u >= 0 && u < cols && v >= 0 && v < rows) {
            const int iu = (int)u, iv = (int)v;
            const long si = (long)k * rows * cols + (long)iv * cols + iu;
            b = bgr8[si * 3 + 0]; g = bgr8[si * 3 + 1]; r = bgr8[si * 3 + 2];
            const double du = (double)((u - cx) / fx), dv = (double)((v - cy) / fy);
            dd = (uint16_t)(depth8[si] * sqrt(1 + du * du + dv * dv));
        }
        const unsigned y = (b * 4899 + g * 9617 + r * 1868 + (1 << 13)) >> 14;
        s_pk[cl][lane] = dd | (y << 16);
        s_bgr[cl][lane] = b | (g << 8) | (r << 16);
    }
    __syncthreads();
    const int tr = threadIdx.x >> 2, c0 = (threadIdx.x & 3) * 4;
    const int grow = ty * STT_R + tr;
    if (grow >= H) return;
    const long i0 = (long)grow * W + tx * STT_C + c0;
    unsigned pk4[4], px[12];
#pragma unroll
    for (int e = 0; e < 4; ++e) {
        pk4[e] = s_pk[c0 + e][tr];
        const unsigned q = s_bgr[c0 + e][tr];
        px[3 * e] = q & 255; px[3 * e + 1] = (q >> 8) & 255; px[3 * e + 2] = q >> 16;
    }
    uint3 wb;
    wb.x = px[0] | (px[1] << 8) | (px[2] << 16) | (px[3] << 24);
    wb.y = px[4] | (px[5] << 8) | (px[6] << 16) | (px[7] << 24);
    wb.z = px[8] | (px[9] << 8) | (px[10] << 16) | (px[11] << 24);
    *reinterpret_cast<uint3*>(sph_bgr + 3 * i0) = wb;
    *reinterpret_cast<uint2*>(sph_depth + i0) = make_uint2((pk4[0] & 0xffffu) | (pk4[1] << 16),
                                                            (pk4[2] & 0xffffu) | (pk4[3] << 16));
    float2 o[4];
#pragma unroll
    for (int e = 0; e < 4; ++e)
        o[e] = make_float2((float)(pk4[e] >> 16) * (float)(1. / 255), (float)(pk4[e] & 0xffffu) * 0.001f);
    *reinterpret_cast<float4*>(p0 + i0) = make_float4(o[0].x, o[0].y, o[1].x, o[1].y);
    *reinterpret_cast<float4*>(p0 + i0 + 2) = make_float4(o[2].x, o[2].y, o[3].x, o[3].y);
    *reinterpret_cast<uint4*>(pk + i0) = make_uint4(pk4[0], pk4[1], pk4[2], pk4[3]);
}

__device__ __forceinline__ int refl101(int p, int n) {
    p = p < 0 ? -p : p;
    return p >= n ? 2 * n - p - 2 : p;
}

struct LvF2 {
    const float2* p;
    __device__ __forceinline__ float g(long i) const { return p[i].x; }
    __device__ __forceinline__ float d(long i) const { return p[i].y; }
    __device__ __forceinline__ float2 gd(long i) const { return p[i]; }
};
struct LvPk {
    const uint32_t* p;
    __device__ __forceinline__ float g(long i) const { return (float)(p[i] >> 16) * (float)(1. / 255); }
    __device__ __forceinline__ float d(long i) const { return (float)(p[i] & 0xffffu) * 0.001f; }
    __device__ __forceinline__ float2 gd(long i) const {
        const uint32_t v = p[i];
        return make_float2((float)(v >> 16) * (float)(1. / 255), (float)(v & 0xffffu) * 0.001f);
    }
};

template <class IN>
__global__ void k_pyramid(const IN in_all, int R, int C, float2* __restrict__ out_all, float min_d, float max_d,
                          int nimg) {
    const int dr = R / 2, dc = C / 2;
    const unsigned per = (unsigned)(dr * dc), n = per * (unsigned)nimg;
    for (unsigned j = blockIdx.x * blockDim.x + threadIdx.x; j < n; j += gridDim.x * blockDim.x) {
        const unsigned img = nimg > 1 ? j / per : 0u;
        const unsigned i = j - img * per;
        const long in0 = (long)img * R * C;
        float2* out = out_all + (long)img * per;
        const int y = (int)(i / (unsigned)dc), x = (int)(i - (unsigned)y * dc);
        const int sx = 2 * x;
        const int xa = refl101(sx - 2, C), xb = refl101(sx - 1, C), xd = refl101(sx + 1, C), xe = refl101(sx + 2, C);
        float h[5];
#pragma unroll
        for (int k = 0; k < 5; ++k) {
            const int yy = refl101(2 * y - 2 + k, R);
            const long s = in0 + (long)yy * C;
            const float a = in_all.g(s + xa), b = in_all.g(s + xb), c = in_all.g(s + sx), d = in_all.g(s + xd),
                        e = in_all.g(s + xe);
            h[k] = c * 6 + (b + d) * 4 + a + e;
        }
        float t0 = h[0] + h[4];
        const float t1 = (h[1] + h[3]) + h[2];
        t0 = t0 + (h[2] + h[2]);
        t0 = t0 + t1 * 4.f;
        const float gray = t0 * (1.f / 256);
        float av = 0.f; unsigned nv = 0;
        const long s0 = in0 + (long)(2 * y) * C + sx;
        const long s1 = s0 + C;
        const float z0 = in_all.d(s0), z1 = in_all.d(s0 + 1), z2 = in_all.d(s1), z3 = in_all.d(s1 + 1);
        if (z0 > min_d && z0 < max_d) { av += z0; ++nv; }
        if (z1 > min_d && z1 < max_d) { av += z1; ++nv; }
        if (z2 > min_d && z2 < max_d) { av += z2; ++nv; }
        if (z3 > min_d && z3 < max_d) { av += z3; ++nv; }
        out[i] = make_float2(gray, nv > 0 ? av / nv : 0.f);
    }
}

__device__ __forceinline__ float harm(float fl, float f, float fr) {
    if ((f > fr && f < fl) || (f < fr && f > fl)) return 2.f / (1 / (fr - f) + 1 / (f - fl));
    return 0.f;
}

__global__ void k_gradient(const float2* __restrict__ p0, int R, int C, float4* __restrict__ tg, int nimg,
                           int mask_seams) {
    const long per = (long)R * C, n = per * nimg;
    const int ws = C / 8;
    for (long i = blockIdx.x * (long)blockDim.x + threadIdx.x; i < n; i += (long)gridDim.x * blockDim.x) {
        const long li = i % per;
        const int r = (int)(li / C), c = (int)(li - (long)r * C);
        float4 o = make_float4(0.f, 0.f, 0.f, 0.f);
        const int m = ws > 0 ? c % ws : 1;
        const bool seam = mask_seams && ws > 0 && (c >= ws - 1) && (c < 7 * ws + 1) && (m == 0 || m == ws - 1);
        if (!seam && r >= 1 && r < R - 1 && c >= 1 && c < C - 1) {
            const float2 f = p0[i], fl = p0[i - 1], fr = p0[i + 1], fu = p0[i - C], fd = p0[i + C];
            o.x = harm(fl.x, f.x, fr.x);
            o.y = harm(fu.x, f.x, fd.x);
            o.z = harm(fl.y, f.y, fr.y);
            o.w = harm(fu.y, f.y, fd.y);
        }
        tg[i] = o;
    }
}

struct GradLevels {
    const float2* p0[R360_MAX_PYR];
    const uint32_t* pk0;
    float4* tg[R360_MAX_PYR];
    int rows[R360_MAX_PYR], cols[R360_MAX_PYR];
    int blk0[R360_MAX_PYR + 1];
    int nl;
};

constexpr int GRAD_PPT = 4;

template <class IN>
__device__ __forceinline__ void gradient_run(const IN p0, int i0, int R, int C, float4* __restrict__ tg) {
    const int ws = C / 8;
    const int n = R * C;
    int r = i0 / C, c = i0 - r * C;
#pragma unroll
    for (int k = 0; k < GRAD_PPT; ++k) {
        const int i = i0 + 64 * k;
        if (i >= n) break;
        float4 o = make_float4(0.f, 0.f, 0.f, 0.f);
        const int m = ws > 0 ? c % ws : 1;
        const bool seam = ws > 0 && (c >= ws - 1) && (c < 7 * ws + 1) && (m == 0 || m == ws - 1);
        if (!seam && r >= 1 && r < R - 1 && c >= 1 && c < C - 1) {
            const float2 f = p0.gd(i), fl = p0.gd(i - 1), fr = p0.gd(i + 1), fu = p0.gd(i - C), fd = p0.gd(i + C);
            o.x = harm(fl.x, f.x, fr.x);
            o.y = harm(fu.x, f.x, fd.x);
            o.z = harm(fl.y, f.y, fr.y);
            o.w = harm(fu.y, f.y, fd.y);
        }
        tg[i] = o;
        c += 64;
        while (c >= C) { c -= C; ++r; }
    }
}

__global__ void k_gradient_levels(GradLevels G) {
    int l = 0;
    while (l + 1 < G.nl && (int)blockIdx.x >= G.blk0[l + 1]) ++l;
    const int R = G.rows[l], C = G.cols[l];
    const int i0 = (int)((blockIdx.x - G.blk0[l]) * blockDim.x * GRAD_PPT + (threadIdx.x & ~63u) * GRAD_PPT +
                         (threadIdx.x & 63u));
    if (i0 >= R * C) return;
    if (l == 0 && G.pk0) gradient_run(LvPk{G.pk0}, i0, R, C, G.tg[0]);
    else gradient_run(LvF2{G.p0[l]}, i0, R, C, G.tg[l]);
}

__global__ void k_sensor_level0(const uint8_t* __restrict__ bgr8, const uint16_t* __restrict__ depth8, long n,
                                float2* __restrict__ p0, uint32_t* __restrict__ pk) {
    for (long i = blockIdx.x * (long)blockDim.x + threadIdx.x; i < n; i += (long)gridDim.x * blockDim.x) {
        const int b = bgr8[3 * i], g = bgr8[3 * i + 1], r = bgr8[3 * i + 2];
        const int y = (b * 4899 + g * 9617 + r * 1868 + (1 << 13)) >> 14;
        p0[i] = make_float2((float)y * (float)(1. / 255), (float)depth8[i] * 0.001f);
        if (pk) pk[i] = depth8[i] | ((unsigned)y << 16);
    }
}

inline int grid_for(long n) {
    long b = (n + TPB - 1) / TPB;
    return (int)(b < 8192 ? (b > 0 ? b : 1) : 8192);
}

}

int launch_undistort(r360_frame* f) {
    const r360_calib* c = f->calib;
    const long n = (long)R360_NUM_SENSORS * f->rows * f->cols;
    const bool apply = c->has_intrinsics && c->clams.width == f->cols && c->clams.height == f->rows;
    if (f->cols % 4 == 0) {
        hipLaunchKernelGGL(k_undistort4, dim3(grid_for(n / 4)), dim3(TPB), 0, f->ctx->stream, f->d_depth, f->d_depth_m,
                           f->rows, f->cols, c->clams.d_mult, c->clams.d_counts, c->clams.nx, c->clams.bin_w,
                           c->clams.bin_h, c->clams.num_bins, c->clams.bin_depth, apply ? 1 : 0);
        R360_HIP(hipGetLastError());
        return 0;
    }
    hipLaunchKernelGGL(k_undistort, dim3(grid_for(n)), dim3(TPB), 0, f->ctx->stream, f->d_depth, f->d_depth_m, f->rows,
                       f->cols, c->clams.d_mult, c->clams.d_counts, c->clams.nx, c->clams.bin_w, c->clams.bin_h,
                       c->clams.num_bins, c->clams.bin_depth, apply ? 1 : 0);
    R360_HIP(hipGetLastError());
    return 0;
}

int launch_stitch(r360_frame* f) {
    const r360_calib* c = f->calib;
    const long n = (long)f->sph_rows * f->sph_cols;
    if (hipEvent_t e = f->bgr_wait()) R360_HIP(hipStreamWaitEvent(f->ctx->stream, e, 0));
    const int slot = timing_begin(f->ctx, "k_stitch");
    static const int form = R360_KNOB("R360_STITCH", 0);
    if (f->sph_cols % STT_C == 0 && form != 4)
        hipLaunchKernelGGL(k_stitch_t, dim3((f->sph_cols / STT_C) * ((f->sph_rows + STT_R - 1) / STT_R)), dim3(256), 0,
                           f->ctx->stream, f->d_bgr, f->d_depth, f->rows, f->cols, f->sph_rows, f->sph_cols,
                           c->d_st_sinphi, c->d_st_cosphi, c->d_st_sinth, c->d_st_costh, c->d_rt_inv, c->K[0], c->K[4],
                           c->K[6], c->K[7], f->d_sph_bgr, f->d_sph_depth, f->lv[0].p0, f->lv[0].pk);
    else if (f->sph_cols % 4 == 0)
        hipLaunchKernelGGL(k_stitch4, dim3(grid_for(n / 4)), dim3(TPB), 0, f->ctx->stream, f->d_bgr, f->d_depth,
                           f->rows, f->cols, f->sph_rows, f->sph_cols, c->d_st_sinphi, c->d_st_cosphi, c->d_st_sinth,
                           c->d_st_costh, c->d_rt_inv, c->K[0], c->K[4], c->K[6], c->K[7], f->d_sph_bgr,
                           f->d_sph_depth, f->lv[0].p0, f->lv[0].pk);
    else
        hipLaunchKernelGGL(k_stitch, dim3(grid_for(n)), dim3(TPB), 0, f->ctx->stream, f->d_bgr, f->d_depth, f->rows,
                           f->cols, f->sph_rows, f->sph_cols, c->d_st_sinphi, c->d_st_cosphi, c->d_st_sinth,
                           c->d_st_costh, c->d_rt_inv, c->K[0], c->K[4], c->K[6], c->K[7], f->d_sph_bgr,
                           f->d_sph_depth, f->lv[0].p0, f->lv[0].pk);
    timing_end(f->ctx, slot);
    R360_HIP(hipGetLastError());
    return 0;
}

constexpr int SRC_PPT = 16, SRC_TPB = R360_SRC_BLOCK / SRC_PPT;

struct SrcGrid { int blk0[R360_MAX_PYR + 1]; int nl; };
__device__ __forceinline__ void src_block(const SrcGrid& G, int& level, int& b) {
    const int bid = blockIdx.x;
    level = 0;
    while (level + 1 < G.nl && bid >= G.blk0[level + 1]) ++level;
    b = bid - G.blk0[level];
}

__device__ __forceinline__ bool src_valid(float d, float min_d, float max_d) { return min_d < d && d < max_d; }

__global__ void __launch_bounds__(SRC_TPB) k_src_count(const SrcLevel* __restrict__ L, SrcGrid G, float min_d, float max_d,
                                                      int* __restrict__ cnt, int stride) {
    int lvl, bx;
    src_block(G, lvl, bx);
    const SrcLevel S = L[lvl];
    const long n = (long)S.rows * S.cols;
    const long b0 = (long)bx * R360_SRC_BLOCK;
    if (b0 >= n) return;
    int c = 0;
#pragma unroll
    for (int k = 0; k < SRC_PPT; ++k) {
        const long i = b0 + k * SRC_TPB + threadIdx.x;
        c += (i < n && src_valid(S.p0[i].y, min_d, max_d)) ? 1 : 0;
    }
    __shared__ int sh[SRC_TPB / 64];
    for (int o = 32; o > 0; o >>= 1) c += __shfl_xor(c, o, 64);
    if ((threadIdx.x & 63) == 0) sh[threadIdx.x >> 6] = c;
    __syncthreads();
    if (threadIdx.x == 0) {
        int t = 0;
        for (int w = 0; w < SRC_TPB / 64; ++w) t += sh[w];
        cnt[lvl * stride + bx] = t;
    }
}

__global__ void __launch_bounds__(SRC_TPB) k_src_compact(const SrcLevel* __restrict__ L, SrcGrid G, float min_d,
                                                        float max_d, const int* __restrict__ cnt, int stride,
                                                        int* __restrict__ npts) {
    int lvl, bx;
    src_block(G, lvl, bx);
    const SrcLevel S = L[lvl];
    const long n = (long)S.rows * S.cols;
    const long b0 = (long)bx * R360_SRC_BLOCK;
    if (b0 >= n) return;
    __shared__ int sh[SRC_TPB / 64 + 1];
    int base = 0;
    for (int b = threadIdx.x; b < bx; b += SRC_TPB) base += cnt[lvl * stride + b];
    for (int o = 32; o > 0; o >>= 1) base += __shfl_xor(base, o, 64);
    if ((threadIdx.x & 63) == 0) sh[threadIdx.x >> 6] = base;
    __syncthreads();
    base = 0;
    for (int w = 0; w < SRC_TPB / 64; ++w) base += sh[w];
    __syncthreads();
    __shared__ int s_cnt[SRC_PPT][SRC_TPB / 64];
    const int lane = threadIdx.x & 63, wid = threadIdx.x >> 6;
    const unsigned long long lt = lane ? (~0ull >> (64 - lane)) : 0ull;
    float2 a[SRC_PPT];
    unsigned long long m[SRC_PPT];
#pragma unroll
    for (int k = 0; k < SRC_PPT; ++k) {
        const long i = b0 + (long)k * SRC_TPB + threadIdx.x;
        a[k] = i < n ? S.p0[i] : make_float2(0.f, 0.f);
        m[k] = __ballot(i < n && src_valid(a[k].y, min_d, max_d));
    }
    if (lane == 0)
#pragma unroll
        for (int k = 0; k < SRC_PPT; ++k) s_cnt[k][wid] = __popcll(m[k]);
    __syncthreads();
    int pos = base;
#pragma unroll
    for (int k = 0; k < SRC_PPT; ++k) {
        int before = pos, row = 0;
#pragma unroll
        for (int w = 0; w < SRC_TPB / 64; ++w) {
            const int cw = s_cnt[k][w];
            before += w < wid ? cw : 0;
            row += cw;
        }
        if ((m[k] >> lane) & 1ull) {
            const long i = b0 + (long)k * SRC_TPB + threadIdx.x;
            const int r = (int)(i / S.cols), cc = (int)(i - (long)r * S.cols);
            const float d = a[k].y;
            S.pts[before + __popcll(m[k] & lt)] =
                make_float4(d * S.sinphi[r], -d * S.cosphi[r] * S.sinth[cc], -d * S.cosphi[r] * S.costh[cc], a[k].x);
        }
        pos += row;
    }
    if (bx == (int)((n - 1) / R360_SRC_BLOCK) && threadIdx.x == SRC_TPB - 1) npts[lvl] = pos;
}

int launch_sphere_level0(r360_frame* f) {
    const long n = (long)f->sph_rows * f->sph_cols;
    hipLaunchKernelGGL(k_sensor_level0, dim3(grid_for(n)), dim3(TPB), 0, f->ctx->stream, f->d_sph_bgr, f->d_sph_depth,
                       n, f->lv[0].p0, f->lv[0].pk);
    R360_HIP(hipGetLastError());
    return 0;
}

int launch_pyramid(r360_frame* f) {
    const float min_d = 0.3f, max_d = 6.0f;
    if ((long)f->lv[0].rows * f->lv[0].cols > 0x7fffffffL - 4096) {
        r360_set_error("sphere of %d x %d pixels is too large", f->lv[0].rows, f->lv[0].cols);
        return -1;
    }
    static const bool pyr_f2 = R360_KNOB("R360_PYR_F2", 0) != 0;
    for (int l = 1; l < f->n_levels; ++l) {
        const long n = (long)f->lv[l].rows * f->lv[l].cols;
        if (l == 1 && f->lv[0].pk && !pyr_f2)
            hipLaunchKernelGGL(k_pyramid<LvPk>, dim3(grid_for(n)), dim3(TPB), 0, f->ctx->stream, LvPk{f->lv[0].pk},
                               f->lv[0].rows, f->lv[0].cols, f->lv[1].p0, min_d, max_d, 1);
        else
            hipLaunchKernelGGL(k_pyramid<LvF2>, dim3(grid_for(n)), dim3(TPB), 0, f->ctx->stream, LvF2{f->lv[l - 1].p0},
                               f->lv[l - 1].rows, f->lv[l - 1].cols, f->lv[l].p0, min_d, max_d, 1);
    }
    {
        GradLevels GL{};
        GL.nl = f->n_levels;
        GL.pk0 = pyr_f2 ? nullptr : f->lv[0].pk;
        for (int l = 0; l < f->n_levels; ++l) {
            GL.p0[l] = f->lv[l].p0;
            GL.tg[l] = f->lv[l].tg;
            GL.rows[l] = f->lv[l].rows;
            GL.cols[l] = f->lv[l].cols;
            GL.blk0[l + 1] = GL.blk0[l] + (int)(((long)f->lv[l].rows * f->lv[l].cols + TPB * GRAD_PPT - 1) / (TPB * GRAD_PPT));
        }
        hipLaunchKernelGGL(k_gradient_levels, dim3(GL.blk0[f->n_levels]), dim3(TPB), 0, f->ctx->stream, GL);
    }
    static const int pf_env = R360_KNOB("R360_ICP_PF", -1);
    const bool skip_ok = !f->compact_all && !(pf_env == 4 || pf_env == 5);
    unsigned need = 0;
    for (int l = 0; l < f->n_levels; ++l) {
        static const bool coarse_pf5 = R360_KNOB("R360_COARSE_PF5", 0) != 0;
        const bool streamed = l == 0 && f->lv[0].pk ? f->lv[0].cols % 64 == 0 : f->lv[l].cols >= 64 && !coarse_pf5;
        if (!skip_ok || !streamed) need |= 1u << l;
    }
    f->compacted = need;
    return launch_src_compaction(f, need);
}

int launch_src_compaction(r360_frame* f, unsigned levels) {
    const float min_d = 0.3f, max_d = 6.0f;
    int l1 = 0;
    for (int l = 0; l < f->n_levels; ++l)
        if ((levels >> l) & 1u) l1 = l + 1;
    if (l1 == 0) return 0;
    SrcGrid G{};
    G.nl = l1;
    for (int l = 0; l < l1; ++l)
        G.blk0[l + 1] = G.blk0[l] + (((levels >> l) & 1u) ? (int)(((long)f->lv[l].rows * f->lv[l].cols + R360_SRC_BLOCK - 1) /
                                                                      R360_SRC_BLOCK) : 0);
    const dim3 g(G.blk0[l1]);
    hipLaunchKernelGGL(k_src_count, g, dim3(SRC_TPB), 0, f->ctx->stream, f->d_src_levels, G, min_d, max_d, f->d_src_cnt,
                       f->src_blocks);
    hipLaunchKernelGGL(k_src_compact, g, dim3(SRC_TPB), 0, f->ctx->stream, f->d_src_levels, G, min_d, max_d,
                       f->d_src_cnt, f->src_blocks, f->d_npts);
    R360_HIP(hipGetLastError());
    return 0;
}

int launch_sensor_pyramid(r360_frame* f) {
    const float min_d = 0.3f, max_d = 6.0f;
    if (!f->n_slevels) {
        int R = f->rows, C = f->cols, nl = 0;
        while (nl < R360_MAX_PYR) {
            f->sp[nl].rows = R; f->sp[nl].cols = C;
            R360_HIP(hipMalloc(&f->sp[nl].p0, sizeof(float2) * 8 * (size_t)R * C));
            R360_HIP(hipMalloc(&f->sp[nl].tg, sizeof(float4) * 8 * (size_t)R * C));
            ++nl;
            if ((R & 1) || (C & 1) || R < 8 || C < 8) break;
            R /= 2; C /= 2;
        }
        f->n_slevels = nl;
    }
    hipStream_t st = f->ctx->stream;
    const long n0 = 8L * f->rows * f->cols;
    if (n0 > 0x7fffffffL) {
        r360_set_error("sensor images of %d x %d pixels are too large", f->rows, f->cols);
        return -1;
    }
    if (hipEvent_t e = f->bgr_wait()) R360_HIP(hipStreamWaitEvent(st, e, 0));
    hipLaunchKernelGGL(k_sensor_level0, dim3(grid_for(n0)), dim3(TPB), 0, st, f->d_bgr, f->d_depth, n0, f->sp[0].p0,
                       (uint32_t*)nullptr);
    for (int l = 1; l < f->n_slevels; ++l) {
        const long n = 8L * f->sp[l].rows * f->sp[l].cols;
        hipLaunchKernelGGL(k_pyramid<LvF2>, dim3(grid_for(n)), dim3(TPB), 0, st, LvF2{f->sp[l - 1].p0}, f->sp[l - 1].rows,
                           f->sp[l - 1].cols, f->sp[l].p0, min_d, max_d, 8);
    }
    for (int l = 0; l < f->n_slevels; ++l) {
        const long n = 8L * f->sp[l].rows * f->sp[l].cols;
        hipLaunchKernelGGL(k_gradient, dim3(grid_for(n)), dim3(TPB), 0, st, f->sp[l].p0, f->sp[l].rows, f->sp[l].cols,
                           f->sp[l].tg, 8, 0);
    }
    R360_HIP(hipGetLastError());
    return 0;
}
```

### rgbd360_amd/csrc/kernels/icp_kernels.hip

```cpp
#include <cstdio>
#include <type_traits>
#include "../r360_internal.h"
#include "../libm_f32.h"

namespace {

#ifndef R360_ICP_TPB
#define R360_ICP_TPB 256
#endif
#ifndef R360_PK_ACC
#define R360_PK_ACC 0
#endif
#ifndef R360_ICP_MINB
#define R360_ICP_MINB 5
#endif
constexpr int TPB = R360_ICP_TPB;
constexpr int NW = TPB / 64;
constexpr int RG = TPB / 16;
static_assert(!R360_GROUP_SUM || R360_TICKET_GROUPS == RG, "R360_GROUP_SUM needs R360_TICKET_GROUPS == TPB / 16");
static_assert(NW >= 3, "the GN step needs at least 3 waves per workgroup (R360_ICP_TPB >= 192)");

struct Pose12 { float R[9]; float t[3]; };

struct Gather {
// ... 1963 lines not shown
    R360_HIP(hipMalloc(&dH, sizeof(double) * 36 * (size_t)n));
    R360_HIP(hipMalloc(&dg, sizeof(double) * 6 * (size_t)n));
    R360_HIP(hipMalloc(&dx, sizeof(double) * 6 * (size_t)n));
    R360_HIP(hipMemcpy(dH, H, sizeof(double) * 36 * (size_t)n, hipMemcpyHostToDevice));
    R360_HIP(hipMemcpy(dg, g, sizeof(double) * 6 * (size_t)n, hipMemcpyHostToDevice));
    hipLaunchKernelGGL(k_solve6, dim3(n), dim3(64), 0, 0, dH, dg, n, dx);
    R360_HIP(hipGetLastError());
    R360_HIP(hipMemcpy(x, dx, sizeof(double) * 6 * (size_t)n, hipMemcpyDeviceToHost));
    (void)hipFree(dH); (void)hipFree(dg); (void)hipFree(dx);
    return 0;
}

extern "C" int r360_rank6(const float* M, int n, int* ranks) {
    if (!M || !ranks || n <= 0) { r360_set_error("r360_rank6: bad arguments"); return -2; }
    float* dM;
    int* dr;
    R360_HIP(hipMalloc(&dM, sizeof(float) * 36 * (size_t)n));
    R360_HIP(hipMalloc(&dr, sizeof(int) * (size_t)n));
    R360_HIP(hipMemcpy(dM, M, sizeof(float) * 36 * (size_t)n, hipMemcpyHostToDevice));
    hipLaunchKernelGGL(k_rank6, dim3(n), dim3(64), 0, 0, dM, n, dr);
    R360_HIP(hipGetLastError());
    R360_HIP(hipMemcpy(ranks, dr, sizeof(int) * (size_t)n, hipMemcpyDeviceToHost));
    (void)hipFree(dM); (void)hipFree(dr);
    return 0;
}

extern "C" int r360_rn_check(unsigned n, unsigned seed, unsigned long long out[2]) {
    unsigned long long* d;
    R360_HIP(hipMalloc(&d, 16));
    R360_HIP(hipMemset(d, 0, 16));
    hipLaunchKernelGGL(k_rn_check, dim3(1024), dim3(256), 0, 0, n, seed, d);
    R360_HIP(hipGetLastError());
    R360_HIP(hipMemcpy(out, d, 16, hipMemcpyDeviceToHost));
    (void)hipFree(d);
    return 0;
}

extern "C" int r360_proj_check(const float* X, const float* Y, const float* Z, int n, int nRows, int nCols,
                               unsigned long long* mismatches, unsigned long long* fallbacks) {
    return proj_check(X, Y, Z, n, nullptr, nRows, nCols, mismatches, fallbacks);
}

extern "C" int r360_proj_check_pose(const float* lx, const float* ly, const float* lz, int n, const float pose[16],
                                    int nRows, int nCols, unsigned long long* mismatches,
                                    unsigned long long* fallbacks) {
    return proj_check(lx, ly, lz, n, pose, nRows, nCols, mismatches, fallbacks);
}

#ifdef R360_STAMPS
extern "C" int r360_debug_block_stamps(unsigned long long* out, int n) {
    if (n > 8192) n = 8192;
    R360_HIP(hipDeviceSynchronize());
    R360_HIP(hipMemcpyFromSymbol(out, HIP_SYMBOL(g_blk_stamps), sizeof(unsigned long long) * 8192 * 3));
    return n;
}
#endif

template <int M, int PF>
static int launch_pass(r360_ctx* ctx, int nb, int njobs, const IcpJobs& jobs, const LevelBufs& Ls,
                        const LevelTrig& T, const IcpConst& C, int first, int eval_only, bool top) {
    void (*kern)(const IcpJobs, const float*, const float*, const float*, const float*, int, int, IcpConst, int, int,
                 unsigned long long*, const uint8_t*) = nullptr;
    if (C.occ) {
        constexpr int PFO = PF >= 4 ? 3 : PF;
        if constexpr (PFO == 0 || PFO == 3 || R360_EXPERIMENTS)
            kern = C.occ == 1 ? k_icp_pass<M, PFO, 0, 1> : k_icp_pass<M, PFO, 0, 2>;
    } else if constexpr (PF == 5 || R360_EXPERIMENTS) {
        kern = top ? k_icp_pass<M, PF, 1, 0> : k_icp_pass<M, PF, 0, 0>;
    } else if constexpr (PF == 6) {
        kern = k_icp_pass<M, PF, 1, 0>;
    } else if constexpr (PF == 8 || PF == 9) {
        kern = k_icp_pass<M, PF, 0, 0>;
    }
    if (!kern) {
        r360_set_error("k_icp_pass: form PF %d (occlusion %d, top %d) is not in this build", PF, C.occ, (int)top);
        return -1;
    }
    hipLaunchKernelGGL(kern, dim3(nb, njobs), dim3(TPB), 0, ctx->stream, jobs, T.sinphi, T.cosphi, T.sinth,
                       T.costh, Ls.rows, Ls.cols, C, first, eval_only, ctx->d_ktime, ctx->occ_flags);
    return 0;
}

int ensure_defer(r360_ctx* ctx, long n_pixels) {
    const long need = n_pixels + (long)ctx->partials_cap * TPB;
    if (ctx->defer_cap >= need) return 0;
    R360_HIP(hipSetDevice(ctx->device));
    R360_HIP(hipStreamSynchronize(ctx->stream));
    if (ctx->d_defer) R360_HIP(hipFree(ctx->d_defer));
    ctx->d_defer = nullptr;
    ctx->defer_cap = 0;
    R360_HIP(hipMalloc(&ctx->d_defer, sizeof(int) * need));
    ctx->defer_cap = need;
    return 0;
}

int ensure_batch(r360_ctx* ctx, int n, long n_pixels) {
    const long dneed = n_pixels + (long)ctx->partials_cap * TPB;
    if (ctx->batch_cap >= n && ctx->bdefer_cap >= dneed) return 0;
    const int cap = n > ctx->batch_cap ? n : ctx->batch_cap;
    const long dcap = dneed > ctx->bdefer_cap ? dneed : ctx->bdefer_cap;
    R360_HIP(hipSetDevice(ctx->device));
    R360_HIP(hipStreamSynchronize(ctx->stream));
    (void)hipFree(ctx->d_bstate); (void)hipFree(ctx->d_bpartials); (void)hipFree(ctx->d_bgticket);
    (void)hipFree(ctx->d_bdefer); (void)hipHostFree(ctx->h_bstate);
    ctx->d_bstate = nullptr; ctx->d_bpartials = nullptr; ctx->d_bgticket = nullptr; ctx->d_bdefer = nullptr;
    ctx->h_bstate = nullptr;
    ctx->batch_cap = 0; ctx->bdefer_cap = 0;
    const size_t tk = (size_t)R360_TICKET_GROUPS * R360_TICKET_STRIDE;
    R360_HIP(hipMalloc(&ctx->d_bstate, sizeof(IcpState) * cap));
    R360_HIP(hipMalloc(&ctx->d_bpartials, sizeof(double) * 32 * (size_t)ctx->partials_cap * cap));
    R360_HIP(hipMalloc(&ctx->d_bgticket, sizeof(unsigned) * tk * cap));
    R360_HIP(hipMemsetAsync(ctx->d_bgticket, 0, sizeof(unsigned) * tk * cap, ctx->stream));
    R360_HIP(hipMalloc(&ctx->d_bdefer, sizeof(int) * (size_t)dcap * cap));
    R360_HIP(hipHostMalloc(&ctx->h_bstate, sizeof(IcpState) * cap, hipHostMallocDefault));
    ctx->batch_cap = cap;
    ctx->bdefer_cap = dcap;
    return 0;
}

struct PassGrid { int pf, nb; };
static PassGrid pass_grid(const r360_ctx* ctx, const LevelBufs& Ls, int occ, int njobs = 1, bool batched = false,
                          bool pts = false) {
    static const int pf_env = R360_KNOB("R360_ICP_PF", -1);
    static const int cap_env = R360_KNOB("R360_ICP_CAP", -1);
    static const int cus = [] {
        int dev = 0, n = 0;
        (void)hipGetDevice(&dev);
        (void)hipDeviceGetAttribute(&n, hipDeviceAttributeMultiprocessorCount, dev);
        return n;
    }();
    const int npx = Ls.rows * Ls.cols;
    const bool pk_ok = Ls.pk != nullptr && Ls.cols % 64 == 0;
    static const bool coarse_pf5 = R360_KNOB("R360_COARSE_PF5", 0) != 0;
    const bool img_ok = !pk_ok && Ls.cols >= 64 && !coarse_pf5;
    const int pf_img = pk_ok ? 6 : img_ok ? (Ls.cols % 64 == 0 ? 8 : 9) : 5;
    const int pf_dflt = occ ? ((Ls.cols % 64 == 0) ? 3 : 0) : (batched || !pts ? pf_img : 5);
    const bool env_ok = pf_env >= 0 && !(pf_env >= 4 && occ) && !((pf_env == 6 || pf_env == 7 || pf_env == 10) && !pk_ok) &&
                        !(pf_env == 8 && Ls.cols % 64 != 0) && !(pf_env == 9 && Ls.cols < 64);
    const int pf = R360_EXPERIMENTS && env_ok ? pf_env : pf_dflt;
    static const int cap_batch_env = R360_KNOB("R360_ICP_CAP_BATCH", -1);
    int cap = cap_env > 0 ? cap_env : 2 * cus;
    if (batched) cap = cap_batch_env > 0 ? cap_batch_env : cus;
    static const int tot_env = R360_KNOB("R360_ICP_WG_TOTAL", -1);
    if (tot_env > 0) cap = ((tot_env / (njobs > 0 ? njobs : 1) + 7) / 8) * 8;
    if (cap > ctx->partials_cap - R360_TICKET_GROUPS) cap = ctx->partials_cap - R360_TICKET_GROUPS;
    static const int pxt_env = R360_KNOB("R360_ICP_PXT", -1);
    const int pxt = pxt_env > 0 ? pxt_env : (batched ? 8 : 1);
    int nb = pf == 1 ? icp_blocks_for(npx) : (npx + TPB * pxt - 1) / (TPB * pxt);
    if (nb > cap) nb = cap;
    if (nb < 1) nb = 1;
    return {pf, nb};
}

static long defer_need(int npx, int nb) {
    const long stride = (long)nb * TPB;
    return (long)nb * (TPB / 64) * (((npx + stride - 1) / stride) * 64);
}

static int launch_jobs(r360_ctx* ctx, const IcpJobs& jobs, int njobs, const LevelBufs& Ls, const LevelTrig& T,
                       int level, int method, const IcpConst& C0, int first, int eval_only, const PassGrid& G) {
    IcpConst C = C0;
    if (++ctx->icp_seq == 0) ++ctx->icp_seq;
    C.seq = ctx->icp_seq;
    const char* name = level == 0 ? "k_icp_pass_L0" : "k_icp_pass";
    const int slot = timing_begin(ctx, name);
    const int pf = G.pf, nb = G.nb;
    const bool top = level == 0;
#if R360_EXPERIMENTS
#define R360_LAUNCH_EXP(M)                                                                               \
        else if (pf == 1) rc = launch_pass<M, 1>(ctx, nb, njobs, jobs, Ls, T, C, first, eval_only, top); \
        else if (pf == 2) rc = launch_pass<M, 2>(ctx, nb, njobs, jobs, Ls, T, C, first, eval_only, top); \
        else if (pf == 4) rc = launch_pass<M, 4>(ctx, nb, njobs, jobs, Ls, T, C, first, eval_only, top); \
        else if (pf == 7) rc = launch_pass<M, 7>(ctx, nb, njobs, jobs, Ls, T, C, first, eval_only, top); \
        else if (pf == 10) rc = launch_pass<M, 10>(ctx, nb, njobs, jobs, Ls, T, C, first, eval_only, top);
#else
#define R360_LAUNCH_EXP(M)
#endif
#define R360_LAUNCH(M)                                                                                   \
    do {                                                                                                 \
        if (pf == 3) rc = launch_pass<M, 3>(ctx, nb, njobs, jobs, Ls, T, C, first, eval_only, top);      \
        else if (pf == 5) rc = launch_pass<M, 5>(ctx, nb, njobs, jobs, Ls, T, C, first, eval_only, top); \
        else if (pf == 6) rc = launch_pass<M, 6>(ctx, nb, njobs, jobs, Ls, T, C, first, eval_only, top); \
        else if (pf == 8) rc = launch_pass<M, 8>(ctx, nb, njobs, jobs, Ls, T, C, first, eval_only, top); \
        else if (pf == 9) rc = launch_pass<M, 9>(ctx, nb, njobs, jobs, Ls, T, C, first, eval_only, top); \
        R360_LAUNCH_EXP(M)                                                                               \
        else rc = launch_pass<M, 0>(ctx, nb, njobs, jobs, Ls, T, C, first, eval_only, top);              \
    } while (0)
    int rc = 0;
    if (method == R360_PHOTO_CONSISTENCY) R360_LAUNCH(R360_PHOTO_CONSISTENCY);
    else if (method == R360_DEPTH_CONSISTENCY) R360_LAUNCH(R360_DEPTH_CONSISTENCY);
    else R360_LAUNCH(R360_PHOTO_DEPTH);
#undef R360_LAUNCH
#undef R360_LAUNCH_EXP
    timing_end(ctx, slot);
    if (rc) return rc;
    R360_HIP(hipGetLastError());
    return 0;
}

int launch_icp_jobs(r360_ctx* ctx, const IcpJobs& jobs, int n, const r360_frame* geom, int level, int method,
                    const IcpConst& C, int first, int eval_only) {
    if (C.occ) { r360_set_error("batched passes: occlusion variants run one alignment per launch"); return -2; }
    if (n < 1 || n > R360_MAX_BATCH) { r360_set_error("batched passes: %d jobs (1..%d)", n, R360_MAX_BATCH); return -2; }
    const LevelBufs& Ls = geom->lv[level];
    const PassGrid G = pass_grid(ctx, Ls, 0, n, true);
    if (G.pf >= 3 && ctx->bdefer_cap < defer_need(Ls.rows * Ls.cols, G.nb)) {
        r360_set_error("batched passes: deferred-pixel queues not sized for %d pixels", Ls.rows * Ls.cols);
        return -1;
    }
    return launch_jobs(ctx, jobs, n, Ls, geom->calib->trig[level], level, method, C, first, eval_only, G);
}

int launch_icp_levels_batch(r360_ctx* ctx, const IcpJobs& jobs, int n, const r360_frame* geom, int level, int method,
                            const IcpConst& C0, int passes) {
#if !R360_EXPERIMENTS
    (void)ctx; (void)jobs; (void)n; (void)geom; (void)level; (void)method; (void)C0; (void)passes;
    return 1;
#else
    static const int coarse_wg = R360_KNOB("R360_COARSE_WG", 64);
    static const int coarse_min = R360_KNOB("R360_COARSE_MIN_LEVEL", 1);
    static const bool persist = R360_KNOB("R360_COARSE_PERSIST", 0) != 0;
    if (level == 0 || level < coarse_min || C0.occ || !persist || !R360_PERSIST_BUILT) return 1;
    if (n < 1 || n > R360_MAX_BATCH) { r360_set_error("batched passes: %d jobs (1..%d)", n, R360_MAX_BATCH); return -2; }
    const LevelBufs& Ls = geom->lv[level];
    PassGrid G = pass_grid(ctx, Ls, 0, n, true);
    if (G.pf != 8 && G.pf != 9) return 1;
    if (G.nb > coarse_wg) G.nb = coarse_wg;
    if (ctx->bdefer_cap < defer_need(Ls.rows * Ls.cols, G.nb)) {
        r360_set_error("batched passes: deferred-pixel queues not sized for %d pixels", Ls.rows * Ls.cols);
        return -1;
    }
    const LevelTrig& T = geom->calib->trig[level];
    IcpConst C = C0;
    if (++ctx->icp_seq == 0) ++ctx->icp_seq;
    C.seq = ctx->icp_seq;
    void (*kern)(const IcpJobs, const float*, const float*, const float*, const float*, int, int, IcpConst, int,
                 unsigned long long*) = nullptr;
    auto pick = [&](auto m) {
        constexpr int M = decltype(m)::value;
        kern = G.pf == 8 ? k_icp_levels_batch<M, 8> : k_icp_levels_batch<M, 9>;
    };
    if (method == R360_PHOTO_CONSISTENCY) pick(std::integral_constant<int, R360_PHOTO_CONSISTENCY>{});
    else if (method == R360_DEPTH_CONSISTENCY) pick(std::integral_constant<int, R360_DEPTH_CONSISTENCY>{});
    else pick(std::integral_constant<int, R360_PHOTO_DEPTH>{});
    const int slot = timing_begin(ctx, "k_icp_levels");
    hipLaunchKernelGGL(kern, dim3(G.nb, n), dim3(TPB), 0, ctx->stream, jobs, T.sinphi, T.cosphi, T.sinth, T.costh,
                       Ls.rows, Ls.cols, C, passes, ctx->d_ktime);
    timing_end(ctx, slot);
    R360_HIP(hipGetLastError());
    return 0;
#endif
}

template <int M, int PF, int TOP>
static int level_blocks_per_cu() {
    static const int n = [] {
        int b = 0;
        if (hipOccupancyMaxActiveBlocksPerMultiprocessor(&b, k_icp_level<M, PF, TOP>, TPB, 0) != hipSuccess) b = 0;
        return b;
    }();
    return n;
}

static int level_blocks_per_cu(int method, int pf) {
    auto by = [&](auto m) {
        constexpr int M = decltype(m)::value;
        return pf == 6 ? level_blocks_per_cu<M, R360_LEVEL_PF0, 1>() : level_blocks_per_cu<M, 5, 0>();
    };
    if (method == R360_PHOTO_CONSISTENCY) return by(std::integral_constant<int, R360_PHOTO_CONSISTENCY>{});
    if (method == R360_DEPTH_CONSISTENCY) return by(std::integral_constant<int, R360_DEPTH_CONSISTENCY>{});
    return by(std::integral_constant<int, R360_PHOTO_DEPTH>{});
}

bool icp_level_persist_ok(r360_ctx* ctx, const r360_frame* src, int level, int method) {
    if (!R360_PERSIST_BUILT) return false;
    const LevelBufs& Ls = src->lv[level];
    const PassGrid G = pass_grid(ctx, Ls, 0, 1, false, (src->compacted >> level) & 1u);
    if (G.pf != 5 && G.pf != 6) return false;
    if (G.pf >= 3 && ctx->defer_cap < defer_need(Ls.rows * Ls.cols, G.nb)) return false;
    int dev = 0, cus = 0;
    if (hipGetDevice(&dev) != hipSuccess || hipDeviceGetAttribute(&cus, hipDeviceAttributeMultiprocessorCount, dev) != hipSuccess)
        return false;
    const int per_cu = level_blocks_per_cu(method, G.pf);
    return per_cu >= 2 && G.nb <= (per_cu - 1) * cus;
}

int launch_icp_level_persist(r360_ctx* ctx, const r360_frame* trg, const r360_frame* src, int level, int method,
                             const IcpConst& C0, int passes) {
    const LevelBufs& Ls = src->lv[level];
    const LevelBufs& Lt = trg->lv[level];
    const LevelTrig& T = src->calib->trig[level];
    const PassGrid G = pass_grid(ctx, Ls, 0, 1, false, (src->compacted >> level) & 1u);
    if (C0.occ || (G.pf != 5 && G.pf != 6) || !R360_PERSIST_BUILT) {
        r360_set_error("persistent level launch: plain pass forms only");
        return -1;
    }
    IcpJobs jobs;
    IcpJob& J = jobs.j[0];
    J.src = Ls.p0; J.trg = Lt.p0; J.tg = Lt.tg; J.pts = Ls.pts; J.npts = src->d_npts + level;
    J.spk = Ls.pk; J.tpk = Lt.pk;
    J.S = ctx->d_state; J.partials = ctx->d_partials; J.gcnt = ctx->d_gticket; J.dq = ctx->d_defer;
    IcpConst C = C0;
    if (++ctx->icp_seq == 0) ++ctx->icp_seq;
    C.seq = ctx->icp_seq;
    const int slot = timing_begin(ctx, level == 0 ? "k_icp_level_L0" : "k_icp_level");
    void (*kern)(const IcpJobs, const float*, const float*, const float*, const float*, int, int, IcpConst, int,
// ... 74 lines not shown
```

### rgbd360_amd/csrc/r360_internal.h

```cpp
#pragma once
#include <atomic>
#include <hip/hip_runtime.h>
#include <stdint.h>
#include <memory>
#include <string>
#include <thread>
#include <vector>
#include "../../include/rgbd360_hip.h"

#define R360_PI 3.14159265359

#ifndef R360_EXPERIMENTS
#define R360_EXPERIMENTS 0
#endif
#if R360_EXPERIMENTS
#include <cstdlib>
#define R360_KNOB(name, dflt) (std::getenv(name) ? std::atoi(std::getenv(name)) : (dflt))
#define R360_KNOB_STR(name) (std::getenv(name))
#else
#define R360_KNOB(name, dflt) (dflt)
#define R360_KNOB_STR(name) ((const char*)nullptr)
#endif

void r360_set_error(const char* fmt, ...);
// ... 276 lines not shown
struct VoxSlot;
struct r360_ctx {
    MapState vmap;
    r360_plane_queue* plane_q = nullptr;
    int device = 0;
    hipStream_t stream = nullptr;
    bool stream_borrowed = false;
    hipEvent_t wait_ev = nullptr;
    hipStream_t mstream = nullptr;
    hipEvent_t mwait_ev = nullptr;
    std::atomic<long long> host_ns[6] = {};
    IcpState* d_state = nullptr;
    double* d_partials = nullptr;
    unsigned* d_gticket = nullptr;
    int* d_defer = nullptr;
    long defer_cap = 0;
    unsigned long long* d_ktime = nullptr;
    long occ_cap = 0;
    int* occ_tgt = nullptr;
    float* occ_dinv = nullptr;
    uint8_t* occ_flags = nullptr;
    int* occ_cnt = nullptr;
    int* occ_off = nullptr;
    int* occ_list = nullptr;
    int* occ_bsum = nullptr;
    int partials_cap = 0;
    unsigned icp_seq = 0;
    struct AlignGraph { std::vector<uintptr_t> key; hipGraphExec_t exec = nullptr; unsigned long long used = 0; };
    std::vector<AlignGraph> graphs;
    unsigned long long graph_clock = 0;
    hipStream_t cap_stream = nullptr;
    struct PlaneGraph { std::string key; hipGraphExec_t exec = nullptr; unsigned long long used = 0; };
    std::vector<PlaneGraph> plane_graphs;
    IcpState* h_state = nullptr;
    int timing = 0;
    r360_ctx* stats_sibling = nullptr;
    int persist_levels = 0;
    int persist_held = 0;
    int async_persist = 0;
    bool join_help = true;
    bool split_upload = true;
    hipStream_t up_stream = nullptr;
    hipEvent_t up_ev = nullptr;
    std::vector<hipEvent_t> ev_pool;
    int ev_used = 0;
    struct TimedLaunch { std::string name; int a, b; };
    std::vector<TimedLaunch> pending;
    struct Acc { double ms = 0; long n = 0; };
    std::vector<std::pair<std::string, Acc>> acc;
    int async_nL = 0, async_pending = 0;
    double align_t0 = 0, align_est = 0;
    int batch_cap = 0;
    long bdefer_cap = 0;
    IcpState* d_bstate = nullptr;
    double* d_bpartials = nullptr;
    unsigned* d_bgticket = nullptr;
    int* d_bdefer = nullptr;
    IcpState* h_bstate = nullptr;
    int batch_n = 0, batch_pending = 0;
    std::vector<hipEvent_t> sync_ev;
    IcpState* d_pin_state = nullptr;
    double* d_pin_partials = nullptr;
    IcpState* h_pin_state = nullptr;
    int pin_pending = 0;
    struct RobotJob* d_rob_jobs = nullptr;
    struct RobotJob* h_rob_jobs = nullptr;
    double* d_rob_partials = nullptr;
    double* d_rob_sums = nullptr;
    double* h_rob_sums = nullptr;
    unsigned* d_rob_tickets = nullptr;
    struct RobotOut* d_rob_out = nullptr;
    struct RobotOut* h_rob_out = nullptr;
    int match_cap = 0;
    r360_match_params match{};
    std::atomic<long> match_calls{0}, match_truncated{0}, match_nodes_max{0};
    float* d_match_desc = nullptr;
    uint8_t* d_unary = nullptr;
    unsigned long long* d_bin = nullptr;
    uint8_t* h_unary = nullptr;
    unsigned long long* h_bin = nullptr;
    VoxCell* d_vhash = nullptr;
    long vhash_cap = 0;
    int* d_vlist = nullptr;
    int* d_vcnt = nullptr;
    long vlist_cap = 0, vcnt_cap = 0;
    std::vector<VoxSlot> bvox;
    int reg_pending = 0, reg_good = 0;
    float reg_info[36];
};

struct ClamsDev {
    int width = 0, height = 0, bin_w = 0, bin_h = 0, nx = 0, ny = 0, num_bins = 0;
    double bin_depth = 2.0;
    float* d_mult = nullptr;
    float* d_counts = nullptr;
};

struct r360_calib {
    r360_ctx* ctx = nullptr;
    int rows = 0, cols = 0;
    float rt[8][16];
    float rt_inv[8][16];
    float K[9];
    bool has_intrinsics = false;
    ClamsDev clams;
    int sph_rows = 0, sph_cols = 0;
    float* d_st_sinphi = nullptr;
    float* d_st_cosphi = nullptr;
    float* d_st_sinth = nullptr;
    float* d_st_costh = nullptr;
    float* d_rt_inv = nullptr;
    float* d_rt = nullptr;
    int n_levels = 0;
    LevelTrig trig[R360_MAX_PYR];
};

struct SphereCloudHost {
    int width = 0, height = 0;
    std::vector<float> xyz;
    std::vector<uint32_t> rgba;
};

struct r360_frame {
    r360_ctx* ctx = nullptr;
    const r360_calib* calib = nullptr;
    int rows = 0, cols = 0, sph_rows = 0, sph_cols = 0, n_levels = 0;
    uint8_t* d_bgr = nullptr;
    hipEvent_t bgr_ev = nullptr;
    bool bgr_split = false;
    hipEvent_t bgr_wait() const { return bgr_split ? bgr_ev : nullptr; }
    uint16_t* d_depth = nullptr;
    float* d_depth_m = nullptr;
    int* d_npts = nullptr;
    int* d_src_cnt = nullptr;
    SrcLevel* d_src_levels = nullptr;
    int src_blocks = 0;
    uint8_t* d_sph_bgr = nullptr;
    uint16_t* d_sph_depth = nullptr;
    LevelBufs lv[R360_MAX_PYR];
    LevelBufs sp[R360_MAX_PYR];
    int n_slevels = 0;
    std::atomic<unsigned> built{0};
    PlaneBufs pl;
    PbMapHost* pbmap = nullptr;
    uint64_t timestamp = 0;
    unsigned compacted = 0;
    bool compact_all = true;
    SphereCloudHost* sphere_cloud = nullptr;
    std::atomic<unsigned> build_gen{0};
};

hipStream_t capture_stream(r360_ctx* ctx);
int launch_undistort(r360_frame* f);
int launch_stitch(r360_frame* f);
int launch_pyramid(r360_frame* f);
int launch_src_compaction(r360_frame* f, unsigned levels);
constexpr int R360_CU_MASK_WORDS = 8;
bool r360_cu_mask(int device, int for_queue, uint32_t* mask);
int launch_sphere_level0(r360_frame* f);
int launch_sensor_pyramid(r360_frame* f);
struct PinJobs { int sensor[8]; int n; };
constexpr int R360_PIN_MAX_BLOCKS = 256;
int launch_pin_level(r360_ctx* ctx, const r360_frame* trg, const r360_frame* src, int level, int method,
                     const IcpConst& C, const float K[4], const PinJobs& J, int first, int eval_only);
struct RobotJob {
    const float2* src;
    const float2* trg;
    const float4* tg;
    int rows, cols;
    float fx, fy, ox, oy, inv_fx, inv_fy;
    double fxd, fyd, oxd, oyd, inv_fxd, inv_fyd;
    float Mrel[16];
    float Rt[16], P[16], Rti[16];
};
constexpr int R360_ROBOT_MAX_JOBS = 8 * R360_MAX_PYR;
constexpr int R360_ROBOT_MAX_BLOCKS = 256;
constexpr int TPB_ROBOT = 256;
struct RobotGrid { int block0[R360_ROBOT_MAX_JOBS + 1]; int njobs; };
struct RobotOut {
    float info[36], grad[6];
    double error[8];
    int ran[8], n_visible[8], n_error[8];
    int ok, illposed_level, any, pad;
};
int launch_robot(r360_ctx* ctx, const RobotJob* d_jobs, const RobotGrid& grid, int method, const IcpConst& C,
                 int finalize_levels);
int launch_icp_level(r360_ctx* ctx, const r360_frame* trg, const r360_frame* src, int level,
                     int method, const IcpConst& C, int first, int eval_only);
int launch_icp_jobs(r360_ctx* ctx, const IcpJobs& jobs, int n, const r360_frame* geom, int level, int method,
                    const IcpConst& C, int first, int eval_only);
int icp_blocks_for(int n_pixels);
bool icp_level_persist_ok(r360_ctx* ctx, const r360_frame* src, int level, int method);
int launch_icp_levels_batch(r360_ctx* ctx, const IcpJobs& jobs, int n, const r360_frame* geom, int level, int method,
                            const IcpConst& C, int passes);
int launch_icp_level_persist(r360_ctx* ctx, const r360_frame* trg, const r360_frame* src, int level, int method,
                             const IcpConst& C, int passes);
int ensure_defer(r360_ctx* ctx, long n_pixels);
int ensure_batch(r360_ctx* ctx, int n, long n_pixels);
int ctx_wait_frames(r360_ctx* ctx, r360_frame* const* frames, int n);
struct PlaneGeom { int rows, cols, w, h, sd_max; long grid_cells; };
PlaneGeom plane_geom(const r360_frame* f);
int launch_cloud_normals(const PlaneBatch& B, int F, const PlaneGeom& G, hipStream_t st, r360_ctx* tctx);
int launch_segmentation(const PlaneBatch& B, int F, const PlaneGeom& G, hipStream_t st, r360_ctx* tctx,
                        const hipEvent_t* bgr_ev);
int launch_rgb(const PlaneBatch& B, int F, const PlaneGeom& G, hipStream_t st);
int launch_segmentation_geom(const PlaneBatch& B, int F, const PlaneGeom& G, hipStream_t st, r360_ctx* tctx);
int launch_segmentation_model(const PlaneBatch& B, int F, const PlaneGeom& G, hipStream_t st, r360_ctx* tctx);
int launch_plane_publish(const PlaneBatch& B, int F, hipStream_t st);
struct VoxScratch { VoxCell* vhash; unsigned long long cap; int* vlist; int* vcnt; };
void vox_scratch_need(const PlaneGeom& G, long* cells, long* entries, long* groups);
struct VoxSlot { VoxScratch v{nullptr, 0, nullptr, nullptr}; long cells = 0, entries = 0, groups = 0; };
int vox_slot_reserve(VoxSlot& s, const PlaneGeom& G, hipStream_t st);
void vox_slot_free(VoxSlot& s);
PlaneDev plane_dev(const r360_frame* f, const VoxScratch& vs);
int plane_bufs_alloc(r360_frame* f);
void plane_bufs_free(r360_frame* f);
int planes_enqueue(r360_frame* f);
int planes_spawn_assembly(r360_frame* f);
int plane_queue_create(int device, int max_batch, r360_plane_queue** out);
void plane_queue_destroy(r360_plane_queue* q);
int plane_queue_submit(r360_plane_queue* q, r360_frame* f);
int plane_queue_stats(const r360_plane_queue* q, long* batches, long* frames, int* max_batch_seen);
r360_ctx* plane_queue_ctx(r360_plane_queue* q);
int ctx_vhash_reserve(r360_ctx* ctx, long min_cells, long list_entries, long list_groups);
int planes_finish(r360_frame* f);
int plane_ticket_poll(const std::shared_ptr<struct PlaneTicket>& tk, std::string* err);
void r360_rot_offset(float Ro[16], float Ri[16]);
void r360_mul4(const float* A, const float* B, float* C);
int planes_assemble(r360_frame* f);
void planes_join(r360_frame* f);

int  timing_begin(r360_ctx* ctx, const char* name);
int  ctx_wait(r360_ctx* ctx);
int  event_wait(hipEvent_t e);
void timing_end(r360_ctx* ctx, int slot);
```

Measured before the change: 1735.

## Add lean stitch skipping level-0 float/BGR outputs and fuse pyramid+gradient kernels

Adds a lean stitch variant that writes only the packed level-0 buffer and skips the spherical BGR, depth and float2 level-0 writes, rematerialising them lazily when a reader or a non-packed ICP form needs them. Replaces the per-level pyramid and gradient launches with a tiled kernel that computes level-0 gradients plus level-1 pyramid and gradients from LDS, and a tail kernel that builds up to three further levels per launch. The aim is to cut HBM write traffic and launch count in frame building. In exchange it adds lazy-materialisation state and extra checks in the alignment paths, and a materialisation can force a synchronous re-stitch.

```diff
diff --git a/include/rgbd360_hip.h b/include/rgbd360_hip.h
--- a/include/rgbd360_hip.h
+++ b/include/rgbd360_hip.h
@@ -37,6 +37,7 @@
     R360_BUILD_CLOUD     = 1u << 3,
     R360_BUILD_PLANES    = 1u << 4,
     R360_BUILD_SENSOR_PYRAMID = 1u << 5,
+    R360_BUILT_LEVEL0 = 1u << 8,
 };
 int  r360_frame_create(r360_ctx* ctx, const r360_calib* calib, r360_frame** out);
 void r360_frame_destroy(r360_frame* f);
diff --git a/rgbd360_amd/__init__.py b/rgbd360_amd/__init__.py
--- a/rgbd360_amd/__init__.py
+++ b/rgbd360_amd/__init__.py
@@ -19,6 +19,7 @@
 PHOTO_CONSISTENCY, DEPTH_CONSISTENCY, PHOTO_DEPTH = 0, 1, 2
 BUILD_UNDISTORT, BUILD_SPHERE, BUILD_PYRAMID, BUILD_CLOUD, BUILD_PLANES = 1, 2, 4, 8, 16
 BUILD_SENSOR_PYRAMID = 32
+BUILT_LEVEL0 = 256
 PCD_ASCII, PCD_BINARY, PCD_BINARY_COMPRESSED = 0, 1, 2
 
 
@@ -611,6 +612,11 @@
         fn = lib().r360_frame_build if sync else lib().r360_frame_build_async
         _check(fn(self.h, flags), "r360_frame_build")
 
+    def built(self) -> int:
+        u = C.c_uint()
+        _check(lib().r360_frame_built(self.h, C.byref(u)), "r360_frame_built")
+        return u.value
+
     def undistort(self):
         self.build(BUILD_UNDISTORT)
 
diff --git a/rgbd360_amd/csrc/host/runtime.cpp b/rgbd360_amd/csrc/host/runtime.cpp
--- a/rgbd360_amd/csrc/host/runtime.cpp
+++ b/rgbd360_amd/csrc/host/runtime.cpp
@@ -696,6 +696,7 @@
     const size_t n = (size_t)sph_rows * sph_cols;
     R360_HIP(hipMemcpyAsync(f->d_sph_bgr, bgr, n * 3, hipMemcpyHostToDevice, f->ctx->stream));
     R360_HIP(hipMemcpyAsync(f->d_sph_depth, range_mm, n * 2, hipMemcpyHostToDevice, f->ctx->stream));
+    f->built |= R360_BUILT_LEVEL0;
     if (launch_sphere_level0(f) || launch_pyramid(f) || frame_build_event_record(f)) return -1;
     R360_HIP(hipStreamSynchronize(f->ctx->stream));
     f->built = (f->built & ~(unsigned)(R360_BUILD_SPHERE | R360_BUILD_PYRAMID)) | R360_BUILD_SPHERE | R360_BUILD_PYRAMID;
@@ -732,7 +733,10 @@
         f->sphere_cloud = nullptr;
     }
     if (flags & (R360_BUILD_SPHERE | R360_BUILD_PYRAMID)) {
-        if (launch_stitch(f)) return -1;
+        const bool lean = frame_level0_lean(f);
+        if (launch_stitch(f, lean)) return -1;
+        if (lean) f->built &= ~(unsigned)R360_BUILT_LEVEL0;
+        else f->built |= R360_BUILT_LEVEL0;
         f->built |= R360_BUILD_SPHERE;
     }
     if (flags & R360_BUILD_PYRAMID) {
@@ -744,6 +748,16 @@
         if (launch_sensor_pyramid(f)) return -1;
         f->built |= R360_BUILD_SENSOR_PYRAMID;
     }
+    return 0;
+}
+
+int frame_level0_materialise(r360_frame* f) {
+    const unsigned b = f->built.load();
+    if ((b & R360_BUILT_LEVEL0) || !(b & R360_BUILD_SPHERE) || f->rows <= 0) return 0;
+    if (bind_device(f->ctx->device)) return -1;
+    if (launch_stitch(f, false)) return -1;
+    R360_HIP(hipStreamSynchronize(f->ctx->stream));
+    f->built |= R360_BUILT_LEVEL0;
     return 0;
 }
 
@@ -788,6 +802,7 @@
 extern "C" int r360_frame_get_sphere(r360_frame* f, uint8_t* bgr, uint16_t* depth) {
     CHECK_ARG(f, "null frame");
     CHECK_ARG(f->built & R360_BUILD_SPHERE, "sphere not built");
+    if (frame_level0_materialise(f)) return -1;
     const size_t n = (size_t)f->sph_rows * f->sph_cols;
     R360_HIP(hipStreamSynchronize(f->ctx->stream));
     if (bgr) R360_HIP(hipMemcpy(bgr, f->d_sph_bgr, n * 3, hipMemcpyDeviceToHost));
@@ -829,6 +844,7 @@
     CHECK_ARG(f, "null frame");
     CHECK_ARG(level >= 0 && level < f->n_levels, "level out of range");
     CHECK_ARG(f->built & R360_BUILD_PYRAMID, "pyramid not built");
+    if (level == 0 && frame_level0_materialise(f)) return -1;
     const LevelBufs& L = f->lv[level];
     return copy_level(f, L.p0, L.tg, L.rows, L.cols, rows, cols, gray, depth, gx, gy, dgx, dgy);
 }
@@ -904,6 +920,12 @@
               "non-default min/max depth changes the depth pyramid: not supported in this version");
     CHECK_ARG(ctx->partials_cap >= icp_blocks_for(src->lv[0].rows * src->lv[0].cols), "partials buffer too small");
     return 0;
+}
+
+static int pair_level0_ready(r360_ctx* ctx, r360_frame* trg, r360_frame* src, int occ, bool batched) {
+    if (icp_pass_form(ctx, src, 0, occ, batched) == 6) return 0;
+    if (frame_level0_materialise(trg) || frame_level0_materialise(src)) return -1;
+    return bind_device(ctx->device);
 }
 
 template <class Enqueue>
@@ -987,6 +1009,7 @@
     CHECK_ARG(init, "null init pose");
     CHECK_ARG(method >= 0 && method <= 2, "invalid method");
     CHECK_ARG(occlusion >= 0 && occlusion <= 2, "occlusion must be 0, 1 or 2");
+    if (pair_level0_ready(ctx, trg, src, occlusion, false)) return -1;
     if (ensure_defer(ctx, src->lv[0].rows * src->lv[0].cols)) return -1;
     for (const r360_frame* f : {trg, src})
         if (f->ctx != ctx)
@@ -1121,6 +1144,8 @@
         CHECK_ARG(src[j]->sph_rows == src[0]->sph_rows && src[j]->sph_cols == src[0]->sph_cols,
                   "batched alignments need frames of one sphere size");
     }
+    for (int j = 0; j < n; ++j)
+        if (pair_level0_ready(ctx, trg[j], src[j], 0, true)) return -1;
     if (ensure_batch(ctx, n, (long)src[0]->lv[0].rows * src[0]->lv[0].cols)) return -1;
     std::vector<r360_frame*> fr;
     for (int j = 0; j < n; ++j) { fr.push_back(trg[j]); fr.push_back(src[j]); }
@@ -1194,6 +1219,7 @@
     CHECK_ARG(level >= 0 && level < src->n_levels, "level out of range");
     CHECK_ARG(method >= 0 && method <= 2, "invalid method");
     CHECK_ARG(occ >= 0 && occ <= 2, "occlusion must be 0, 1 or 2");
+    if (level == 0 && pair_level0_ready(ctx, trg, src, occ, false)) return -1;
     if (ensure_defer(ctx, src->lv[level].rows * src->lv[level].cols)) return -1;
     IcpState* h = ctx->h_state;
     memset(h, 0, sizeof(IcpState));
diff --git a/rgbd360_amd/csrc/kernels/frame_kernels.hip b/rgbd360_amd/csrc/kernels/frame_kernels.hip
--- a/rgbd360_amd/csrc/kernels/frame_kernels.hip
+++ b/rgbd360_amd/csrc/kernels/frame_kernels.hip
@@ -184,6 +184,7 @@
 }
 
 constexpr int STT_R = 64, STT_C = 16;
+template <bool LEAN>
 __global__ void __launch_bounds__(256) k_stitch_t(const uint8_t* __restrict__ bgr8, const uint16_t* __restrict__ depth8,
                                                   int rows, int cols, int H, int W, const float* __restrict__ sinphi,
                                                   const float* __restrict__ cosphi, const float* __restrict__ sinth,
@@ -192,7 +193,7 @@
                                                   uint16_t* __restrict__ sph_depth, float2* __restrict__ p0,
                                                   uint32_t* __restrict__ pk) {
     __shared__ uint32_t s_pk[STT_C][STT_R + 1];
-    __shared__ uint32_t s_bgr[STT_C][STT_R + 1];
+    __shared__ uint32_t s_bgr[LEAN ? 1 : STT_C][STT_R + 1];
     const int lane = threadIdx.x & 63, w = threadIdx.x >> 6;
     const int tiles_x = W / STT_C;
     const int tx = blockIdx.x % tiles_x, ty = blockIdx.x / tiles_x;
@@ -223,7 +224,7 @@
         }
         const unsigned y = (b * 4899 + g * 9617 + r * 1868 + (1 << 13)) >> 14;
         s_pk[cl][lane] = dd | (y << 16);
-        s_bgr[cl][lane] = b | (g << 8) | (r << 16);
+        if (!LEAN) s_bgr[cl][lane] = b | (g << 8) | (r << 16);
     }
     __syncthreads();
     const int tr = threadIdx.x >> 2, c0 = (threadIdx.x & 3) * 4;
@@ -232,8 +233,11 @@
     const long i0 = (long)grow * W + tx * STT_C + c0;
     unsigned pk4[4], px[12];
 #pragma unroll
+    for (int e = 0; e < 4; ++e) pk4[e] = s_pk[c0 + e][tr];
+    *reinterpret_cast<uint4*>(pk + i0) = make_uint4(pk4[0], pk4[1], pk4[2], pk4[3]);
+    if (LEAN) return;
+#pragma unroll
     for (int e = 0; e < 4; ++e) {
-        pk4[e] = s_pk[c0 + e][tr];
         const unsigned q = s_bgr[c0 + e][tr];
         px[3 * e] = q & 255; px[3 * e + 1] = (q >> 8) & 255; px[3 * e + 2] = q >> 16;
     }
@@ -250,7 +254,6 @@
         o[e] = make_float2((float)(pk4[e] >> 16) * (float)(1. / 255), (float)(pk4[e] & 0xffffu) * 0.001f);
     *reinterpret_cast<float4*>(p0 + i0) = make_float4(o[0].x, o[0].y, o[1].x, o[1].y);
     *reinterpret_cast<float4*>(p0 + i0 + 2) = make_float4(o[2].x, o[2].y, o[3].x, o[3].y);
-    *reinterpret_cast<uint4*>(pk + i0) = make_uint4(pk4[0], pk4[1], pk4[2], pk4[3]);
 }
 
 __device__ __forceinline__ int refl101(int p, int n) {
@@ -263,9 +266,17 @@
     __device__ __forceinline__ float g(long i) const { return p[i].x; }
     __device__ __forceinline__ float d(long i) const { return p[i].y; }
     __device__ __forceinline__ float2 gd(long i) const { return p[i]; }
+    typedef float2 cell;
+    __device__ __forceinline__ cell raw(long i) const { return p[i]; }
+    static __device__ __forceinline__ float2 val(cell v) { return v; }
 };
 struct LvPk {
     const uint32_t* p;
+    typedef uint32_t cell;
+    __device__ __forceinline__ cell raw(long i) const { return p[i]; }
+    static __device__ __forceinline__ float2 val(cell v) {
+        return make_float2((float)(v >> 16) * (float)(1. / 255), (float)(v & 0xffffu) * 0.001f);
+    }
     __device__ __forceinline__ float g(long i) const { return (float)(p[i] >> 16) * (float)(1. / 255); }
     __device__ __forceinline__ float d(long i) const { return (float)(p[i] & 0xffffu) * 0.001f; }
     __device__ __forceinline__ float2 gd(long i) const {
@@ -339,51 +350,204 @@
     }
 }
 
-struct GradLevels {
-    const float2* p0[R360_MAX_PYR];
-    const uint32_t* pk0;
-    float4* tg[R360_MAX_PYR];
-    int rows[R360_MAX_PYR], cols[R360_MAX_PYR];
-    int blk0[R360_MAX_PYR + 1];
-    int nl;
+__device__ __forceinline__ bool grad_live(int r, int c, int R, int C) {
+    const int ws = C / 8;
+    const int m = ws > 0 ? c % ws : 1;
+    const bool seam = ws > 0 && (c >= ws - 1) && (c < 7 * ws + 1) && (m == 0 || m == ws - 1);
+    return !seam && r >= 1 && r < R - 1 && c >= 1 && c < C - 1;
+}
+
+__device__ __forceinline__ float4 grad_of(float2 f, float2 fl, float2 fr, float2 fu, float2 fd) {
+    return make_float4(harm(fl.x, f.x, fr.x), harm(fu.x, f.x, fd.x), harm(fl.y, f.y, fr.y), harm(fu.y, f.y, fd.y));
+}
+
+__device__ __forceinline__ float pyr_gray(float h0, float h1, float h2, float h3, float h4) {
+    float t0 = h0 + h4;
+    const float t1 = (h1 + h3) + h2;
+    t0 = t0 + (h2 + h2);
+    t0 = t0 + t1 * 4.f;
+    return t0 * (1.f / 256);
+}
+__device__ __forceinline__ float pyr_depth(float z0, float z1, float z2, float z3, float min_d, float max_d) {
+    float av = 0.f; unsigned nv = 0;
+    if (z0 > min_d && z0 < max_d) { av += z0; ++nv; }
+    if (z1 > min_d && z1 < max_d) { av += z1; ++nv; }
+    if (z2 > min_d && z2 < max_d) { av += z2; ++nv; }
+    if (z3 > min_d && z3 < max_d) { av += z3; ++nv; }
+    return nv > 0 ? av / nv : 0.f;
+}
+
+__device__ __forceinline__ int clampi(int p, int n) { return p < 0 ? 0 : (p >= n ? n - 1 : p); }
+
+constexpr int L0_TR = 16, L0_TC = 128, L0_HALO = 4;
+constexpr int L0_SR = L0_TR + 2 * L0_HALO, L0_SC = L0_TC + 2 * L0_HALO;
+constexpr int L0_1R = L0_TR / 2 + 2, L0_1C = L0_TC / 2 + 2;
+constexpr int L0_HR = 2 * L0_1R + 3;
+
+template <class IN>
+__global__ void __launch_bounds__(256) k_prep_l0(const IN in, int R, int C, float4* __restrict__ tg0,
+                                                 float2* __restrict__ p1, float4* __restrict__ tg1, float min_d,
+                                                 float max_d) {
+    __shared__ typename IN::cell s0[L0_SR][L0_SC];
+    __shared__ float sh[L0_HR][L0_1C];
+    __shared__ float2 s1[L0_1R][L0_1C];
+    const int tiles_x = (C + L0_TC - 1) / L0_TC;
+    const int ty = blockIdx.x / tiles_x, tx = blockIdx.x - ty * tiles_x;
+    const int y0 = ty * L0_TR, x0 = tx * L0_TC;
+#pragma unroll 4
+    for (int k = threadIdx.x; k < L0_SR * L0_SC; k += 256) {
+        const int r = k / L0_SC, c = k - r * L0_SC;
+        const int gy = clampi(refl101(y0 - L0_HALO + r, R), R), gx = clampi(refl101(x0 - L0_HALO + c, C), C);
+        s0[r][c] = in.raw((long)gy * C + gx);
+    }
+    __syncthreads();
+    for (int k = threadIdx.x; k < L0_TR * L0_TC; k += 256) {
+        const int r = k / L0_TC, c = k - r * L0_TC;
+        const int gy = y0 + r, gx = x0 + c;
+        if (gy >= R || gx >= C) continue;
+        float4 o = make_float4(0.f, 0.f, 0.f, 0.f);
+        if (grad_live(gy, gx, R, C)) {
+            const int lr = r + L0_HALO, lc = c + L0_HALO;
+            o = grad_of(IN::val(s0[lr][lc]), IN::val(s0[lr][lc - 1]), IN::val(s0[lr][lc + 1]), IN::val(s0[lr - 1][lc]),
+                        IN::val(s0[lr + 1][lc]));
+        }
+        tg0[(long)gy * C + gx] = o;
+    }
+    if (!p1) return;
+    const int dr = R / 2, dc = C / 2, Y0 = y0 / 2, X0 = x0 / 2;
+    for (int k = threadIdx.x; k < L0_HR * L0_1C; k += 256) {
+        const int s = k / L0_1C, j = k - s * L0_1C;
+        const typename IN::cell* row = s0[s] + 2 * j;
+        const float a = IN::val(row[0]).x, b = IN::val(row[1]).x, c = IN::val(row[2]).x, d = IN::val(row[3]).x,
+                    e = IN::val(row[4]).x;
+        sh[s][j] = c * 6 + (b + d) * 4 + a + e;
+    }
+    __syncthreads();
+    for (int k = threadIdx.x; k < L0_1R * L0_1C; k += 256) {
+        const int i = k / L0_1C, j = k - i * L0_1C;
+        const int ly = Y0 - 1 + i, lx = X0 - 1 + j;
+        if (ly < 0 || ly >= dr || lx < 0 || lx >= dc) continue;
+        const float gray = pyr_gray(sh[2 * i][j], sh[2 * i + 1][j], sh[2 * i + 2][j], sh[2 * i + 3][j], sh[2 * i + 4][j]);
+        const typename IN::cell* r0 = s0[2 * i + 2] + 2 * j + 2;
+        const typename IN::cell* r1 = s0[2 * i + 3] + 2 * j + 2;
+        const float2 v = make_float2(gray, pyr_depth(IN::val(r0[0]).y, IN::val(r0[1]).y, IN::val(r1[0]).y,
+                                                     IN::val(r1[1]).y, min_d, max_d));
+        s1[i][j] = v;
+        if (i >= 1 && i <= L0_TR / 2 && j >= 1 && j <= L0_TC / 2) p1[(long)ly * dc + lx] = v;
+    }
+    __syncthreads();
+    for (int k = threadIdx.x; k < (L0_TR / 2) * (L0_TC / 2); k += 256) {
+        const int i = k / (L0_TC / 2), j = k - i * (L0_TC / 2);
+        const int ly = Y0 + i, lx = X0 + j;
+        if (ly >= dr || lx >= dc) continue;
+        float4 o = make_float4(0.f, 0.f, 0.f, 0.f);
+        if (grad_live(ly, lx, dr, dc))
+            o = grad_of(s1[i + 1][j + 1], s1[i + 1][j], s1[i + 1][j + 2], s1[i][j + 1], s1[i + 2][j + 1]);
+        tg1[(long)ly * dc + lx] = o;
+    }
+}
+
+constexpr int TL_R = 16, TL_C = 32;
+constexpr int TL_T = 512;
+constexpr int TL_CR = TL_R / 4 + 2, TL_CC = TL_C / 4 + 2;
+constexpr int TL_BR = 2 * TL_CR + 3, TL_BC = 2 * TL_CC + 3;
+constexpr int TL_AR = 2 * TL_BR + 3, TL_AC = 2 * TL_BC + 3;
+
+struct TailLevels {
+    float2* p0[3];
+    float4* tg[3];
+    int nb;
 };
 
-constexpr int GRAD_PPT = 4;
-
-template <class IN>
-__device__ __forceinline__ void gradient_run(const IN p0, int i0, int R, int C, float4* __restrict__ tg) {
-    const int ws = C / 8;
-    const int n = R * C;
-    int r = i0 / C, c = i0 - r * C;
-#pragma unroll
-    for (int k = 0; k < GRAD_PPT; ++k) {
-        const int i = i0 + 64 * k;
-        if (i >= n) break;
+struct SrcGlobal {
+    const float2* p; int C;
+    __device__ __forceinline__ float2 at(int y, int x) const { return p[(long)y * C + x]; }
+};
+template <int NC>
+struct SrcLds {
+    const float2 (*s)[NC]; int oy, ox;
+    __device__ __forceinline__ float2 at(int y, int x) const { return s[y - oy][x - ox]; }
+};
+
+template <int DR, int DC, bool CLAMP, class SRC>
+__device__ __forceinline__ void tail_step(const SRC src, int Rs, int Cs, int doy, int dox, float* __restrict__ h,
+                                          float2 (*dst)[DC], float2* __restrict__ gout, int ty0, int tx0, int tr, int tc,
+                                          float min_d, float max_d) {
+    const int Rd = Rs / 2, Cd = Cs / 2, sy0 = 2 * doy - 2;
+#pragma unroll 2
+    for (int k = threadIdx.x; k < (2 * DR + 3) * DC; k += TL_T) {
+        const int s = k / DC, j = k - s * DC;
+        int sy = sy0 + s, xd = dox + j;
+        if (CLAMP) { sy = clampi(sy, Rs); xd = clampi(xd, Cd); }
+        else if (sy < 0 || sy >= Rs || xd < 0 || xd >= Cd) continue;
+        const int sx = 2 * xd;
+        const float a = src.at(sy, refl101(sx - 2, Cs)).x, b = src.at(sy, refl101(sx - 1, Cs)).x, c = src.at(sy, sx).x,
+                    d = src.at(sy, refl101(sx + 1, Cs)).x, e = src.at(sy, refl101(sx + 2, Cs)).x;
+        h[k] = c * 6 + (b + d) * 4 + a + e;
+    }
+    __syncthreads();
+#pragma unroll 2
+    for (int k = threadIdx.x; k < DR * DC; k += TL_T) {
+        const int i = k / DC, j = k - i * DC;
+        const int yd = doy + i, xd = dox + j;
+        const bool in = yd >= 0 && yd < Rd && xd >= 0 && xd < Cd;
+        if (!CLAMP && !in) continue;
+        const int yq = CLAMP ? clampi(yd, Rd) : yd, xq = CLAMP ? clampi(xd, Cd) : xd;
+        const float2 z0 = src.at(2 * yq, 2 * xq), z1 = src.at(2 * yq, 2 * xq + 1), z2 = src.at(2 * yq + 1, 2 * xq),
+                     z3 = src.at(2 * yq + 1, 2 * xq + 1);
+        if (CLAMP && !in) continue;
+        float hh[5];
+#pragma unroll
+        for (int t = 0; t < 5; ++t) hh[t] = h[(refl101(2 * yd - 2 + t, Rs) - sy0) * DC + j];
+        const float2 v = make_float2(pyr_gray(hh[0], hh[1], hh[2], hh[3], hh[4]),
+                                     pyr_depth(z0.y, z1.y, z2.y, z3.y, min_d, max_d));
+        dst[i][j] = v;
+        if (yd >= ty0 && yd < ty0 + tr && xd >= tx0 && xd < tx0 + tc) gout[(long)yd * Cd + xd] = v;
+    }
+    __syncthreads();
+}
+
+template <int TR, int TC, int NC>
+__device__ __forceinline__ void tail_grad(const float2 (*s)[NC], int oy, int ox, int R, int C, int ty0, int tx0,
+                                          float4* __restrict__ tg) {
+    for (int k = threadIdx.x; k < TR * TC; k += TL_T) {
+        const int i = k / TC, j = k - i * TC;
+        const int y = ty0 + i, x = tx0 + j;
+        if (y >= R || x >= C) continue;
         float4 o = make_float4(0.f, 0.f, 0.f, 0.f);
-        const int m = ws > 0 ? c % ws : 1;
-        const bool seam = ws > 0 && (c >= ws - 1) && (c < 7 * ws + 1) && (m == 0 || m == ws - 1);
-        if (!seam && r >= 1 && r < R - 1 && c >= 1 && c < C - 1) {
-            const float2 f = p0.gd(i), fl = p0.gd(i - 1), fr = p0.gd(i + 1), fu = p0.gd(i - C), fd = p0.gd(i + C);
-            o.x = harm(fl.x, f.x, fr.x);
-            o.y = harm(fu.x, f.x, fd.x);
-            o.z = harm(fl.y, f.y, fr.y);
-            o.w = harm(fu.y, f.y, fd.y);
-        }
-        tg[i] = o;
-        c += 64;
-        while (c >= C) { c -= C; ++r; }
-    }
-}
-
-__global__ void k_gradient_levels(GradLevels G) {
-    int l = 0;
-    while (l + 1 < G.nl && (int)blockIdx.x >= G.blk0[l + 1]) ++l;
-    const int R = G.rows[l], C = G.cols[l];
-    const int i0 = (int)((blockIdx.x - G.blk0[l]) * blockDim.x * GRAD_PPT + (threadIdx.x & ~63u) * GRAD_PPT +
-                         (threadIdx.x & 63u));
-    if (i0 >= R * C) return;
-    if (l == 0 && G.pk0) gradient_run(LvPk{G.pk0}, i0, R, C, G.tg[0]);
-    else gradient_run(LvF2{G.p0[l]}, i0, R, C, G.tg[l]);
+        if (grad_live(y, x, R, C)) {
+            const int ly = y - oy, lx = x - ox;
+            o = grad_of(s[ly][lx], s[ly][lx - 1], s[ly][lx + 1], s[ly - 1][lx], s[ly + 1][lx]);
+        }
+        tg[(long)y * C + x] = o;
+    }
+}
+
+__global__ void __launch_bounds__(TL_T) k_prep_tail(const float2* __restrict__ base, int R0, int C0, TailLevels T,
+                                                   float min_d, float max_d) {
+    __shared__ float sh[(2 * TL_AR + 3) * TL_AC];
+    __shared__ float2 sa[TL_AR][TL_AC];
+    __shared__ float2 sb[TL_BR][TL_BC];
+    __shared__ float2 sc[TL_CR][TL_CC];
+    const int Ra = R0 / 2, Ca = C0 / 2;
+    const int tiles_x = (Ca + TL_C - 1) / TL_C;
+    const int ty = blockIdx.x / tiles_x, tx = blockIdx.x - ty * tiles_x;
+    const int Yc = ty * (TL_R / 4), Xc = tx * (TL_C / 4);
+    const int cy = Yc - 1, cx = Xc - 1;
+    const int by = 2 * cy - 2, bx = 2 * cx - 2;
+    const int ay = 2 * by - 2, ax = 2 * bx - 2;
+    tail_step<TL_AR, TL_AC, true>(SrcGlobal{base, C0}, R0, C0, ay, ax, sh, sa, T.p0[0], 4 * Yc, 4 * Xc, TL_R, TL_C, min_d,
+                            max_d);
+    tail_grad<TL_R, TL_C>(sa, ay, ax, Ra, Ca, 4 * Yc, 4 * Xc, T.tg[0]);
+    if (T.nb < 2) return;
+    const int Rb = Ra / 2, Cb = Ca / 2;
+    tail_step<TL_BR, TL_BC, false>(SrcLds<TL_AC>{sa, ay, ax}, Ra, Ca, by, bx, sh, sb, T.p0[1], 2 * Yc, 2 * Xc, TL_R / 2,
+                            TL_C / 2, min_d, max_d);
+    tail_grad<TL_R / 2, TL_C / 2>(sb, by, bx, Rb, Cb, 2 * Yc, 2 * Xc, T.tg[1]);
+    if (T.nb < 3) return;
+    tail_step<TL_CR, TL_CC, false>(SrcLds<TL_BC>{sb, by, bx}, Rb, Cb, cy, cx, sh, sc, T.p0[2], Yc, Xc, TL_R / 4, TL_C / 4,
+                            min_d, max_d);
+    tail_grad<TL_R / 4, TL_C / 4>(sc, cy, cx, Rb / 2, Cb / 2, Yc, Xc, T.tg[2]);
 }
 
 __global__ void k_sensor_level0(const uint8_t* __restrict__ bgr8, const uint16_t* __restrict__ depth8, long n,
@@ -421,18 +585,42 @@
     return 0;
 }
 
-int launch_stitch(r360_frame* f) {
+static int stitch_form() {
+    static const int form = R360_KNOB("R360_STITCH", 0);
+    return form;
+}
+
+bool frame_level0_lean(const r360_frame* f) {
+    static const int pf_env = R360_KNOB("R360_ICP_PF", -1);
+    static const bool pyr_f2 = R360_KNOB("R360_PYR_F2", 0) != 0;
+    static const bool lean_on = R360_KNOB("R360_LEAN", 1) != 0;
+    return lean_on && !f->compact_all && !(pf_env == 4 || pf_env == 5) && !pyr_f2 && f->rows > 0 && f->lv[0].pk &&
+           f->lv[0].cols % 64 == 0 && stitch_form() != 4;
+}
+
+int launch_stitch(r360_frame* f, bool lean) {
     const r360_calib* c = f->calib;
     const long n = (long)f->sph_rows * f->sph_cols;
     if (hipEvent_t e = f->bgr_wait()) R360_HIP(hipStreamWaitEvent(f->ctx->stream, e, 0));
     const int slot = timing_begin(f->ctx, "k_stitch");
-    static const int form = R360_KNOB("R360_STITCH", 0);
-    if (f->sph_cols % STT_C == 0 && form != 4)
-        hipLaunchKernelGGL(k_stitch_t, dim3((f->sph_cols / STT_C) * ((f->sph_rows + STT_R - 1) / STT_R)), dim3(256), 0,
-                           f->ctx->stream, f->d_bgr, f->d_depth, f->rows, f->cols, f->sph_rows, f->sph_cols,
-                           c->d_st_sinphi, c->d_st_cosphi, c->d_st_sinth, c->d_st_costh, c->d_rt_inv, c->K[0], c->K[4],
-                           c->K[6], c->K[7], f->d_sph_bgr, f->d_sph_depth, f->lv[0].p0, f->lv[0].pk);
-    else if (f->sph_cols % 4 == 0)
+    const int form = stitch_form();
+    if (lean && !(f->sph_cols % STT_C == 0 && form != 4)) {
+        r360_set_error("lean stitch: the tiled form only");
+        return -1;
+    }
+    if (f->sph_cols % STT_C == 0 && form != 4) {
+        const dim3 grid((f->sph_cols / STT_C) * ((f->sph_rows + STT_R - 1) / STT_R));
+        if (lean)
+            hipLaunchKernelGGL(k_stitch_t<true>, grid, dim3(256), 0, f->ctx->stream, f->d_bgr, f->d_depth, f->rows,
+                               f->cols, f->sph_rows, f->sph_cols, c->d_st_sinphi, c->d_st_cosphi, c->d_st_sinth,
+                               c->d_st_costh, c->d_rt_inv, c->K[0], c->K[4], c->K[6], c->K[7], f->d_sph_bgr,
+                               f->d_sph_depth, f->lv[0].p0, f->lv[0].pk);
+        else
+            hipLaunchKernelGGL(k_stitch_t<false>, grid, dim3(256), 0, f->ctx->stream, f->d_bgr, f->d_depth, f->rows,
+                               f->cols, f->sph_rows, f->sph_cols, c->d_st_sinphi, c->d_st_cosphi, c->d_st_sinth,
+                               c->d_st_costh, c->d_rt_inv, c->K[0], c->K[4], c->K[6], c->K[7], f->d_sph_bgr,
+                               f->d_sph_depth, f->lv[0].p0, f->lv[0].pk);
+    } else if (f->sph_cols % 4 == 0)
         hipLaunchKernelGGL(k_stitch4, dim3(grid_for(n / 4)), dim3(TPB), 0, f->ctx->stream, f->d_bgr, f->d_depth,
                            f->rows, f->cols, f->sph_rows, f->sph_cols, c->d_st_sinphi, c->d_st_cosphi, c->d_st_sinth,
                            c->d_st_costh, c->d_rt_inv, c->K[0], c->K[4], c->K[6], c->K[7], f->d_sph_bgr,
@@ -554,27 +742,26 @@
         return -1;
     }
     static const bool pyr_f2 = R360_KNOB("R360_PYR_F2", 0) != 0;
-    for (int l = 1; l < f->n_levels; ++l) {
-        const long n = (long)f->lv[l].rows * f->lv[l].cols;
-        if (l == 1 && f->lv[0].pk && !pyr_f2)
-            hipLaunchKernelGGL(k_pyramid<LvPk>, dim3(grid_for(n)), dim3(TPB), 0, f->ctx->stream, LvPk{f->lv[0].pk},
-                               f->lv[0].rows, f->lv[0].cols, f->lv[1].p0, min_d, max_d, 1);
+    {
+        const LevelBufs& L0 = f->lv[0];
+        const bool more = f->n_levels > 1;
+        float2* p1 = more ? f->lv[1].p0 : nullptr;
+        float4* tg1 = more ? f->lv[1].tg : nullptr;
+        const dim3 grid(((L0.rows + L0_TR - 1) / L0_TR) * ((L0.cols + L0_TC - 1) / L0_TC));
+        if (L0.pk && !pyr_f2)
+            hipLaunchKernelGGL(k_prep_l0<LvPk>, grid, dim3(256), 0, f->ctx->stream, LvPk{L0.pk}, L0.rows, L0.cols, L0.tg,
+                               p1, tg1, min_d, max_d);
         else
-            hipLaunchKernelGGL(k_pyramid<LvF2>, dim3(grid_for(n)), dim3(TPB), 0, f->ctx->stream, LvF2{f->lv[l - 1].p0},
-                               f->lv[l - 1].rows, f->lv[l - 1].cols, f->lv[l].p0, min_d, max_d, 1);
-    }
-    {
-        GradLevels GL{};
-        GL.nl = f->n_levels;
-        GL.pk0 = pyr_f2 ? nullptr : f->lv[0].pk;
-        for (int l = 0; l < f->n_levels; ++l) {
-            GL.p0[l] = f->lv[l].p0;
-            GL.tg[l] = f->lv[l].tg;
-            GL.rows[l] = f->lv[l].rows;
-            GL.cols[l] = f->lv[l].cols;
-            GL.blk0[l + 1] = GL.blk0[l] + (int)(((long)f->lv[l].rows * f->lv[l].cols + TPB * GRAD_PPT - 1) / (TPB * GRAD_PPT));
-        }
-        hipLaunchKernelGGL(k_gradient_levels, dim3(GL.blk0[f->n_levels]), dim3(TPB), 0, f->ctx->stream, GL);
+            hipLaunchKernelGGL(k_prep_l0<LvF2>, grid, dim3(256), 0, f->ctx->stream, LvF2{L0.p0}, L0.rows, L0.cols, L0.tg,
+                               p1, tg1, min_d, max_d);
+    }
+    for (int l = 1; l + 1 < f->n_levels; l += 3) {
+        TailLevels T{};
+        T.nb = f->n_levels - 1 - l < 3 ? f->n_levels - 1 - l : 3;
+        for (int k = 0; k < T.nb; ++k) { T.p0[k] = f->lv[l + 1 + k].p0; T.tg[k] = f->lv[l + 1 + k].tg; }
+        const LevelBufs& A = f->lv[l + 1];
+        hipLaunchKernelGGL(k_prep_tail, dim3(((A.rows + TL_R - 1) / TL_R) * ((A.cols + TL_C - 1) / TL_C)), dim3(TL_T), 0,
+                           f->ctx->stream, f->lv[l].p0, f->lv[l].rows, f->lv[l].cols, T, min_d, max_d);
     }
     static const int pf_env = R360_KNOB("R360_ICP_PF", -1);
     const bool skip_ok = !f->compact_all && !(pf_env == 4 || pf_env == 5);
@@ -594,6 +781,7 @@
     for (int l = 0; l < f->n_levels; ++l)
         if ((levels >> l) & 1u) l1 = l + 1;
     if (l1 == 0) return 0;
+    if ((levels & 1u) && frame_level0_materialise(f)) return -1;
     SrcGrid G{};
     G.nl = l1;
     for (int l = 0; l < l1; ++l)
diff --git a/rgbd360_amd/csrc/kernels/icp_kernels.hip b/rgbd360_amd/csrc/kernels/icp_kernels.hip
--- a/rgbd360_amd/csrc/kernels/icp_kernels.hip
+++ b/rgbd360_amd/csrc/kernels/icp_kernels.hip
@@ -2139,6 +2139,10 @@
     return {pf, nb};
 }
 
+int icp_pass_form(const r360_ctx* ctx, const r360_frame* src, int level, int occ, bool batched) {
+    return pass_grid(ctx, src->lv[level], occ, 1, batched, !batched && ((src->compacted >> level) & 1u)).pf;
+}
+
 static long defer_need(int npx, int nb) {
     const long stride = (long)nb * TPB;
     return (long)nb * (TPB / 64) * (((npx + stride - 1) / stride) * 64);
diff --git a/rgbd360_amd/csrc/r360_internal.h b/rgbd360_amd/csrc/r360_internal.h
--- a/rgbd360_amd/csrc/r360_internal.h
+++ b/rgbd360_amd/csrc/r360_internal.h
@@ -452,7 +452,10 @@
 
 hipStream_t capture_stream(r360_ctx* ctx);
 int launch_undistort(r360_frame* f);
-int launch_stitch(r360_frame* f);
+int launch_stitch(r360_frame* f, bool lean = false);
+bool frame_level0_lean(const r360_frame* f);
+int frame_level0_materialise(r360_frame* f);
+int icp_pass_form(const r360_ctx* ctx, const r360_frame* src, int level, int occ, bool batched);
 int launch_pyramid(r360_frame* f);
 int launch_src_compaction(r360_frame* f, unsigned levels);
 constexpr int R360_CU_MASK_WORDS = 8;
```

After: 1773 (median of 6 runs). 2.2% higher.
